# JunkyByte/deepcharuco

Hardware: AMD Instinct MI355X
Metric: frames/sec end-to-end (detect+refine) at 320x240; corner-id match vs ref (higher is better)
Workload: dtype f32; 1 GPU; bs=32/GPU x1 GPU(s) = 32 frames of 320x240, full detect+refine pipeline (BASELINE configs[1]); preset=cfg2, batch_per_gpu=32, global_batch=32, height=240, width=320, corner_pool_per_gpu=2048, frames=board, truncated_frames=0, distinct_ids_in_batch=16, parallelism=frames sharded, 1 process/GPU x1

## Files before the change

deepcharuco_amd/_lib.py:

```python
from __future__ import annotations

import ctypes as C
import os
import subprocess
from typing import Optional

_HERE = os.path.dirname(os.path.abspath(__file__))
LIB_PATH = os.environ.get("DCX_LIB") or os.path.join(_HERE, "libdeepcharuco_amd.so")
CSRC = os.path.join(_HERE, "csrc")

_lib: Optional[C.CDLL] = None


class DcxError(RuntimeError):
    def __init__(self, code: int, where: str):
        self.code = code
        try:
            msg = lib().dcx_error_string(code).decode()
        except Exception:
            msg = "?"
        super().__init__(f"{where} failed with code {code}: {msg}")


def build(force: bool = False, verbose: bool = False) -> str:
    cmd = ["make", "-C", CSRC, "-j4"]
    if force:
        subprocess.run(["make", "-C", CSRC, "clean"], check=True, capture_output=not verbose)
    res = subprocess.run(cmd, capture_output=True, text=True)
    if res.returncode != 0:
        raise RuntimeError("building libdeepcharuco_amd.so failed:\n" + res.stdout[-4000:] + res.stderr[-8000:])
    if verbose:
        print(res.stdout)
    return LIB_PATH


_vp, _i, _l, _sz = C.c_void_p, C.c_int, C.c_long, C.c_size_t

SIGNATURES = {
    "dcx_version": (C.c_char_p, []),
    "dcx_error_string": (C.c_char_p, [_i]),
    "dcx_detector_create": (_i, [C.POINTER(_vp), C.POINTER(_vp), _i, _i]),
    "dcx_detector_destroy": (_i, [_vp]),
    "dcx_refiner_create": (_i, [C.POINTER(_vp), C.POINTER(_vp), _i]),
    "dcx_refiner_destroy": (_i, [_vp]),
    "dcx_detector_workspace_bytes": (_sz, [_vp, _i, _i, _i]),
    "dcx_refiner_workspace_bytes": (_sz, [_vp, _i]),
    "dcx_bgr2gray": (_i, [_vp, _l, _i, _i, _i, _i, _vp, _vp]),
    "dcx_bgr2gray_legacy14": (_i, [_vp, _l, _i, _i, _i, _i, _vp, _vp]),
    "dcx_pre_image": (_i, [_vp, _vp, _sz, _vp]),
    "dcx_detector_forward": (_i, [_vp, _vp, _l, _i, _vp, _i, _i, _i, _vp, _sz, _vp, _vp, _vp]),
    "dcx_detector_decode": (_i, [_vp, _i, _i, _i, _vp, _i, _i, _vp, _vp, _vp, _vp, _vp]),
    "dcx_pred_to_keypoints": (_i, [_vp, _vp, _i, _i, _i, _i, _i, _i, _i, _vp, _vp, _vp, _vp, _vp]),
    "dcx_label_to_keypoints": (_i, [_vp, _vp, _i, _i, _i, _i, _i, _vp, _vp, _vp, _vp, _vp]),
    "dcx_build_patch_table": (_i, [_vp, _vp, _i, _i, _vp, _vp, _vp]),
    "dcx_extract_patches_u8": (_i, [_vp, _l, _i, _i, _i, _vp, _vp, _i, _vp, _vp]),
    "dcx_extract_patches_f32": (_i, [_vp, _i, _i, _vp, _vp, _i, _vp, _vp]),
    "dcx_refiner_forward": (_i, [_vp, _vp, _i, _vp, _vp, _vp, _sz, _vp, _vp, _vp, _vp]),
    "dcx_argmax2d": (_i, [_vp, _i, _i, _i, _vp, _vp]),
    "dcx_pipeline_workspace_bytes": (_sz, [_vp, _vp, _i, _i, _i, _i]),
    "dcx_infer_batch": (_i, [_vp, _vp, _vp, _l, _i, _i, _i, _i, _i, _i, _i, _vp, _sz, _vp, _vp, _vp, _vp, _vp, _vp]),
    "dcx_stream_synchronize": (_i, [_vp]),
    "dcx_solve_pnp_pool": (_i, [_vp, _vp, _vp, _vp, _i, _i, _i, _i, C.c_double, C.POINTER(C.c_double), C.POINTER(C.c_double), _i,
                               _vp, _vp, _vp]),
    "dcx_solve_pnp_ransac_workspace_bytes": (_sz, [_i, _i, _i]),
    "dcx_solve_pnp_ransac_pool": (_i, [_vp, _vp, _vp, _vp, _i, _i, _i, _i, C.c_double, C.POINTER(C.c_double), C.POINTER(C.c_double), _i,
                                      _i, C.c_double, _i, C.c_uint, _vp, _sz, _vp, _vp, _vp, _vp, _vp]),
    "dcx_calibrate_workspace_bytes": (_sz, [_i]),
    "dcx_calibrate_pool": (_i, [_vp, _vp, _vp, _vp, _i, _i, _i, _i, C.c_double, _i, _i, _vp, _sz, _vp, _vp,
                               C.POINTER(C.c_double), _vp]),
    "dcx_conv_layer": (_i, [_vp, _i, _i, _i, _i, _vp, _vp, _vp, _vp, _vp, _vp, _i, _i, _i, _i, _i, _i, _vp, _vp]),
    "dcx_nchw_to_c4": (_i, [_vp, _i, _i, _i, _i, _vp, _vp]),
    "dcx_c4_to_nchw": (_i, [_vp, _i, _i, _i, _i, _vp, _vp]),
    "dcx_set_timing": (_i, [_i]),
    "dcx_get_timing": (_i, []),
    "dcx_profile_enabled": (_i, []),
    "dcx_last_timings": (_i, [C.POINTER(C.c_float)]),
    "dcx_conv_pick_name": (C.c_char_p, [_i] * 8),
    "dcx_conv_pick_name_ups": (C.c_char_p, [_i] * 9),
    "dcx_set_deterministic": (_i, [_i]),
    "dcx_get_deterministic": (_i, []),
    "dcx_calibrate_xcd": (_i, [_i, C.POINTER(C.c_float), _vp]),
    "dcx_set_xcd_weights": (_i, [C.POINTER(C.c_float)]),
    "dcx_get_xcd_weights": (_i, [C.POINTER(C.c_float)]),
    "dcx_set_tail_fence": (_i, [_i]),
    "dcx_get_tail_fence": (_i, []),
    "dcx_profile_enable": (_i, [_i]),
    "dcx_profile_count": (_i, []),
    "dcx_profile_filter": (_i, [_i]),
    "dcx_profile_sample": (_i, [_i]),
    "dcx_profile_fetch": (_i, [C.POINTER(_i), C.POINTER(_i), C.POINTER(_i), C.POINTER(C.c_double), C.POINTER(C.c_float), _i]),
    "dcx_profile_kernel_name": (C.c_char_p, [_i]),
    "dcx_profile_clocks": (_i, [C.POINTER(C.c_float), _i]),
    "dcx_profile_probe_words": (_i, [_i, C.POINTER(C.c_ulonglong)]),
}


def lib() -> C.CDLL:
    global _lib
    if _lib is None:
        if not os.path.exists(LIB_PATH):
            raise RuntimeError(
                f"{LIB_PATH} not found: build it with `python -c 'import __graft_entry__ as g; g.build()'` "
                f"or `make -C {CSRC}`. deepcharuco_amd has no CPU / stock-PyTorch fallback.")
        handle = C.CDLL(LIB_PATH)
        for name, (res, args) in SIGNATURES.items():
            fn = getattr(handle, name)
            fn.restype = res
            fn.argtypes = args
        _lib = handle
    return _lib


def csrc_sha256() -> str:
    import hashlib
    h = hashlib.sha256()
    for name in sorted(os.listdir(CSRC)):
        if name.endswith((".hip", ".h")):
            with open(os.path.join(CSRC, name), "rb") as f:
                h.update(name.encode())
                h.update(f.read())
    return h.hexdigest()


def check(rc: int, where: str) -> None:
    if rc != 0:
        raise DcxError(rc, where)


def ptr(t) -> Optional[int]:
    if t is None:
        return None
    return t.data_ptr()


def current_stream() -> int:
    import torch
    return torch.cuda.current_stream().cuda_stream
```

deepcharuco_amd/csrc/dcx_api.hip:

```cpp
#include "dcx_common.h"

#include <math.h>
#include <stdlib.h>
#include <string.h>
#include <new>
#include <vector>

namespace {

constexpr float kBnEps = 1e-5f;

inline size_t align_up(size_t v, size_t a) { return (v + a - 1) / a * a; }


std::vector<float> pack_conv(const float* w, int cout, int cin, int ks, int cout_pad) {
    const int taps = ks * ks, cq = cin / 4;
    std::vector<float> out((size_t)taps * cq * cout_pad * 4, 0.0f);
    for (int o = 0; o < cout; ++o)
        for (int i = 0; i < cin; ++i)
            for (int t = 0; t < taps; ++t)
                out[(((size_t)t * cq + (i >> 2)) * cout_pad + o) * 4 + (i & 3)] = w[((size_t)o * cin + i) * taps + t];
    return out;
}

std::vector<float> pack_conv_wino2(const float* w, int cout, int cin, int cout_pad) {
    const int cq = cin / 4;
    std::vector<float> out((size_t)16 * cq * cout_pad * 4, 0.0f);
    for (int o = 0; o < cout; ++o)
        for (int i = 0; i < cin; ++i) {
            const float* g = w + ((size_t)o * cin + i) * 9;
            float h[4][3], u[4][4];
            for (int kx = 0; kx < 3; ++kx) {
                const float g0 = g[kx], g1 = g[3 + kx], g2 = g[6 + kx];
                h[0][kx] = g0; h[1][kx] = ((g0 + g1) + g2) * 0.5f; h[2][kx] = ((g0 - g1) + g2) * 0.5f; h[3][kx] = g2;
            }
            for (int xi = 0; xi < 4; ++xi) {
                u[xi][0] = h[xi][0]; u[xi][1] = ((h[xi][0] + h[xi][1]) + h[xi][2]) * 0.5f;
                u[xi][2] = ((h[xi][0] - h[xi][1]) + h[xi][2]) * 0.5f; u[xi][3] = h[xi][2];
            }
            for (int pos = 0; pos < 16; ++pos)
                out[(((size_t)pos * cq + (i >> 2)) * cout_pad + o) * 4 + (i & 3)] = u[pos >> 2][pos & 3];
        }
    return out;
}

std::vector<float> pack_conv_ups2(const float* w, int cout, int cin, int cout_pad) {
    const int cq = cin / 4;
    std::vector<float> out((size_t)16 * cq * cout_pad * 4, 0.0f);
    static const int lo[2][2] = {{0, 1}, {0, 2}}, hi[2][2] = {{0, 2}, {1, 2}};
    for (int o = 0; o < cout; ++o)
        for (int i = 0; i < cin; ++i) {
            const float* g = w + ((size_t)o * cin + i) * 9;
            for (int ph = 0; ph < 4; ++ph)
                for (int tap = 0; tap < 4; ++tap) {
                    const int a = ph >> 1, b = ph & 1, dy = tap >> 1, dx = tap & 1;
                    float r[3];
                    for (int kx = 0; kx < 3; ++kx) {
                        r[kx] = g[lo[a][dy] * 3 + kx];
                        for (int ky = lo[a][dy] + 1; ky <= hi[a][dy]; ++ky) r[kx] = r[kx] + g[ky * 3 + kx];
                    }
                    float v = r[lo[b][dx]];
                    for (int kx = lo[b][dx] + 1; kx <= hi[b][dx]; ++kx) v = v + r[kx];
                    out[(((size_t)(ph * 4 + tap) * cq + (i >> 2)) * cout_pad + o) * 4 + (i & 3)] = v;
                }
        }
    return out;
}

std::vector<float> pack_conv_ups2w(const float* w, int cout, int cin, int cout_pad) {
    const int cq = cin / 4;
    const std::vector<float> ph = pack_conv_ups2(w, cout, cin, cout_pad);
    std::vector<float> out((size_t)36 * cq * cout_pad * 4, 0.0f);
    const size_t plane = (size_t)cq * cout_pad * 4;
    for (int p = 0; p < 4; ++p)
        for (size_t e = 0; e < plane; ++e) {
            float wc[2][3];
            for (int dy = 0; dy < 2; ++dy) {
                const float g0 = ph[(size_t)(p * 4 + dy * 2 + 0) * plane + e], g1 = ph[(size_t)(p * 4 + dy * 2 + 1) * plane + e];
                wc[dy][0] = g0; wc[dy][1] = g0 + g1; wc[dy][2] = g1;
            }
            for (int nu = 0; nu < 3; ++nu) {
                out[(size_t)(p * 9 + 0 * 3 + nu) * plane + e] = wc[0][nu];
                out[(size_t)(p * 9 + 1 * 3 + nu) * plane + e] = wc[0][nu] + wc[1][nu];
                out[(size_t)(p * 9 + 2 * 3 + nu) * plane + e] = wc[1][nu];
            }
        }
    return out;
}

void fold_bn(const float* gamma, const float* bbeta, const float* mean, const float* var, int c, int c_pad,
             std::vector<float>& alpha, std::vector<float>& beta) {
    alpha.assign(c_pad, 0.0f);
    beta.assign(c_pad, 0.0f);
    for (int i = 0; i < c; ++i) {
        const float inv = 1.0f / sqrtf(var[i] + kBnEps);
        const float a = gamma[i] * inv;
        alpha[i] = a;
        beta[i] = bbeta[i] - mean[i] * a;
    }
}

std::vector<float> pad_vec(const float* v, int c, int c_pad) {
    std::vector<float> out(c_pad, 0.0f);
    memcpy(out.data(), v, sizeof(float) * c);
    return out;
}

struct DevLayer {
    float* w = nullptr;
    float* w_wino2 = nullptr;
    float* w_ups2w = nullptr;
    float* bias = nullptr;
    float* alpha = nullptr;
    float* beta = nullptr;
    int cin = 0, cout = 0, cout_pad = 0, ks = 3;
};

int upload(const std::vector<float>& h, float** d) {
    DCX_CHECK_HIP(hipMalloc((void**)d, h.size() * sizeof(float)));
    DCX_CHECK_HIP(hipMemcpy(*d, h.data(), h.size() * sizeof(float), hipMemcpyHostToDevice));
    return 0;
}

void free_layer(DevLayer& l) {
    if (l.w) (void)hipFree(l.w);
    if (l.w_wino2) (void)hipFree(l.w_wino2);
    if (l.w_ups2w) (void)hipFree(l.w_ups2w);
    if (l.bias) (void)hipFree(l.bias);
    if (l.alpha) (void)hipFree(l.alpha);
    if (l.beta) (void)hipFree(l.beta);
    l = DevLayer();
}

struct HostConv {
    const float* w; const float* b;
    const float* g; const float* be; const float* mu; const float* var;
};

int make_layer(const HostConv& h, int cin, int cout, int ks, DevLayer* out, bool ups_input = false) {
    DevLayer l;
    l.cin = cin; l.cout = cout; l.ks = ks;
    l.cout_pad = dcx_conv_cout_pad(cout);
    int rc = upload(pack_conv(h.w, cout, cin, ks, l.cout_pad), &l.w);
    if (rc == 0) rc = upload(pad_vec(h.b, cout, l.cout_pad), &l.bias);
    if (rc == 0 && h.g != nullptr) {
        std::vector<float> al, be;
        fold_bn(h.g, h.be, h.mu, h.var, cout, l.cout_pad, al, be);
        for (int i = 0; i < cout; ++i) be[i] = fmaf(h.b[i], al[i], be[i]);
        rc = upload(al, &l.alpha);
        if (rc == 0) rc = upload(be, &l.beta);
        if (rc == 0 && ks == 3) rc = upload(pack_conv_wino2(h.w, cout, cin, l.cout_pad), &l.w_wino2);
        if (rc == 0 && ks == 3 && ups_input) rc = upload(pack_conv_ups2w(h.w, cout, cin, l.cout_pad), &l.w_ups2w);
    }
    if (rc != 0) { free_layer(l); return rc; }
    *out = l;
    return 0;
}

int make_first_layer(const HostConv& h, DevLayer* out) {
    DevLayer l;
    l.cin = 1; l.cout = 64; l.cout_pad = 64; l.ks = 3;
    std::vector<float> w(9 * 64);
    for (int o = 0; o < 64; ++o)
        for (int t = 0; t < 9; ++t) w[t * 64 + o] = h.w[o * 9 + t];
    std::vector<float> al, be;
    fold_bn(h.g, h.be, h.mu, h.var, 64, 64, al, be);
    int rc = upload(w, &l.w);
    if (rc == 0) rc = upload(pad_vec(h.b, 64, 64), &l.bias);
    if (rc == 0) rc = upload(al, &l.alpha);
    if (rc == 0) rc = upload(be, &l.beta);
    if (rc != 0) { free_layer(l); return rc; }
    *out = l;
    return 0;
}

bool g_timing = false;
hipEvent_t g_ev[5];
bool g_ev_ok = false;
int timing_mark(int i, hipStream_t s) {
    if (!g_timing) return 0;
    if (!g_ev_ok) {
        for (auto& e : g_ev) DCX_CHECK_HIP(hipEventCreate(&e));
        g_ev_ok = true;
    }
    DCX_CHECK_HIP(hipEventRecord(g_ev[i], s));
    return 0;
}

}

struct dcx_detector {
    int n_ids = 16;
    DevLayer first;
    DevLayer enc[7];
    DevLayer heads_a;
    DevLayer head_loc, head_ids;
};

struct dcx_refiner {
    DevLayer first;
    DevLayer mid[9];
    DevLayer head_a;
    float* head_w = nullptr;
    float head_b = 0.f;
};

namespace {

struct DetWs {
    size_t buf0, buf1, loc, ids, codes, conf, total;
    int ids_quads;
};
DetWs det_layout(int n_ids, int b, int h, int w) {
    DetWs L;
    const size_t hw = (size_t)h * w, cells = (size_t)(h / 8) * (w / 8);
    L.ids_quads = (n_ids + 1 + 3) / 4;
    size_t off = 0;
    L.buf0 = off; off = align_up(off + (size_t)b * 64 * hw * 4, 256);
    L.buf1 = off; off = align_up(off + (size_t)b * 16 * hw * 4, 256);
    L.loc = off;  off = align_up(off + (size_t)b * 68 * cells * 4, 256);
    L.ids = off;  off = align_up(off + (size_t)b * L.ids_quads * 4 * cells * 4, 256);
    L.codes = off; off = align_up(off + (size_t)b * cells * 4, 256);
    L.conf = off; off = align_up(off + (size_t)b * cells * 8, 256);
    L.total = off;
    return L;
}

struct RefWs {
    size_t buf0, buf1, pval, pidx, total;
};
constexpr int kRefTiles = 32;
RefWs ref_layout(int p) {
    RefWs L;
    size_t off = 0;
    L.buf0 = off; off = align_up(off + (size_t)p * 65536 * 4, 256);
    L.buf1 = off; off = align_up(off + (size_t)p * 65536 * 4, 256);
    L.pval = off; off = align_up(off + (size_t)p * kRefTiles * 4, 256);
    L.pidx = off; off = align_up(off + (size_t)p * kRefTiles * 4, 256);
    L.total = off;
    return L;
}

DcxConvArgs conv_args(const DevLayer& l, const float* in, int n, int in_cq_total, int in_cq_off, int hin, int win,
                      int ups, int pad, float* out, int out_cq_total, const int* n_limit) {
    DcxConvArgs a;
    memset(&a, 0, sizeof(a));
    a.in = in; a.w = l.w; a.w_wino2 = l.w_wino2; a.w_ups2w = l.w_ups2w; a.bias = l.bias; a.alpha = l.alpha; a.beta = l.beta; a.out = out;
    a.n_limit = n_limit;
    a.n = n; a.in_cq_total = in_cq_total; a.in_cq_off = in_cq_off; a.cin = l.cin;
    a.hin = hin; a.win = win; a.ups = ups; a.pad = pad;
    a.ho = (hin << ups) + 2 * pad - (l.ks - 1);
    a.wo = (win << ups) + 2 * pad - (l.ks - 1);
    a.out_cq_total = out_cq_total; a.out_cq_off = 0;
    a.cout_pad = l.cout_pad; a.cout_quads = (l.cout + 3) / 4; a.cout_real = l.cout;
    return a;
}

}

extern "C" const char* dcx_version(void) { return "deepcharuco_amd 0.1 (gfx950, fp32 MFMA)"; }

extern "C" const char* dcx_error_string(int code) {
    switch (code) {
        case 0: return "ok";
        case DCX_E_ARG: return "DCX_E_ARG: null pointer or bad scalar argument";
        case DCX_E_SHAPE: return "DCX_E_SHAPE: unsupported shape (H/W below 8, patches not 24x24, batch x kmax too large, ...)";
        case DCX_E_WS: return "DCX_E_WS: workspace too small";
        case DCX_E_NIDS: return "DCX_E_NIDS: n_ids outside [1, 62] or dust_bin outside [0, 255]";
        default: return code > 0 ? hipGetErrorString((hipError_t)code) : "unknown dcx error";
    }
}

extern "C" int dcx_detector_create(dcx_detector** out, const float* const* t, int n_tensors, int n_ids) {
    if (!out || !t) return DCX_E_ARG;
    if (n_ids < 1 || n_ids > 62) return DCX_E_NIDS;
    if (n_tensors != 64) return DCX_E_ARG;
    for (int i = 0; i < n_tensors; ++i)
        if (!t[i]) return DCX_E_ARG;
    if (const int rc = dcx_xcd_init()) return rc;
    dcx_detector* d = new (std::nothrow) dcx_detector();
    if (!d) return (int)hipErrorOutOfMemory;
    d->n_ids = n_ids;
    auto hc = [&](int base, bool bn) {
        return HostConv{t[base], t[base + 1], bn ? t[base + 2] : nullptr, bn ? t[base + 3] : nullptr,
                        bn ? t[base + 4] : nullptr, bn ? t[base + 5] : nullptr};
    };
    static const int enc_cin[7] = {64, 64, 64, 64, 128, 128, 128};
    static const int enc_cout[7] = {64, 64, 64, 128, 128, 128, 128};
    int rc = make_first_layer(hc(0, true), &d->first);
    for (int i = 0; rc == 0 && i < 7; ++i) rc = make_layer(hc(6 + 6 * i, true), enc_cin[i], enc_cout[i], 3, &d->enc[i]);
    if (rc == 0) {
        const HostConv pa = hc(48, true), da = hc(56, true);
        const size_t wsz = (size_t)256 * 128 * 9;
        std::vector<float> w(2 * wsz), b(512), g(512), be(512), mu(512), var(512);
        memcpy(w.data(), pa.w, wsz * 4); memcpy(w.data() + wsz, da.w, wsz * 4);
        auto cat = [](std::vector<float>& dst, const float* x, const float* y) {
            memcpy(dst.data(), x, 256 * 4); memcpy(dst.data() + 256, y, 256 * 4);
        };
        cat(b, pa.b, da.b); cat(g, pa.g, da.g); cat(be, pa.be, da.be); cat(mu, pa.mu, da.mu); cat(var, pa.var, da.var);
        rc = make_layer(HostConv{w.data(), b.data(), g.data(), be.data(), mu.data(), var.data()}, 128, 512, 3,
                        &d->heads_a);
    }
    if (rc == 0) rc = make_layer(hc(54, false), 256, 65, 1, &d->head_loc);
    if (rc == 0) rc = make_layer(hc(62, false), 256, n_ids + 1, 1, &d->head_ids);
    if (rc != 0) { dcx_detector_destroy(d); return rc; }
    *out = d;
    return 0;
}

extern "C" int dcx_detector_destroy(dcx_detector* d) {
    if (!d) return 0;
    free_layer(d->first);
    for (auto& l : d->enc) free_layer(l);
    free_layer(d->heads_a); free_layer(d->head_loc); free_layer(d->head_ids);
    delete d;
    return 0;
}

extern "C" size_t dcx_detector_workspace_bytes(const dcx_detector* det, int batch, int height, int width) {
    if (!det || batch <= 0 || height <= 0 || width <= 0) return 0;
    return det_layout(det->n_ids, batch, height, width).total;
}

namespace {
int detector_run(const dcx_detector* det, const uint8_t* d_frames_u8, long frame_stride, int pitch, int pix,
                 const float* d_images_f32, int batch, int height, int width, void* d_ws, size_t ws_bytes,
                 bool with_heads, float* d_loc_nchw, float* d_ids_nchw, int32_t* zero_words, int n_zero, void* stream);
}

extern "C" int dcx_detector_forward(const dcx_detector* det, const uint8_t* d_frames_u8, long frame_stride, int pitch,
                                    const float* d_images_f32, int batch, int height, int width, void* d_ws,
                                    size_t ws_bytes, float* d_loc_nchw, float* d_ids_nchw, void* stream) {
    return detector_run(det, d_frames_u8, frame_stride, pitch, DCX_PIX_GRAY8, d_images_f32, batch, height, width, d_ws, ws_bytes, true,
                        d_loc_nchw, d_ids_nchw, nullptr, 0, stream);
}

namespace {
int detector_run(const dcx_detector* det, const uint8_t* d_frames_u8, long frame_stride, int pitch, int pix,
                 const float* d_images_f32, int batch, int height, int width, void* d_ws, size_t ws_bytes,
                 bool with_heads, float* d_loc_nchw, float* d_ids_nchw, int32_t* zero_words, int n_zero, void* stream) {
    if (!det || !d_ws) return DCX_E_ARG;
    if ((d_frames_u8 == nullptr) == (d_images_f32 == nullptr)) return DCX_E_ARG;
    if (batch <= 0 || height < 8 || width < 8) return DCX_E_SHAPE;
    const DetWs L = det_layout(det->n_ids, batch, height, width);
    if (ws_bytes < L.total) return DCX_E_WS;
    hipStream_t s = (hipStream_t)stream;
    char* ws = (char*)d_ws;
    float* buf0 = (float*)(ws + L.buf0);
    float* buf1 = (float*)(ws + L.buf1);
    float* loc = (float*)(ws + L.loc);
    float* ids = (float*)(ws + L.ids);
    const int h = height, w = width;
    int rc;
    const int pt0 = dcx_prof_begin(DCX_PROF_CONV1A, batch, s);
    if (d_frames_u8)
        rc = dcx_launch_conv1_u8(d_frames_u8, frame_stride, pitch, pix, batch, h, w, 1, det->first.w, det->first.bias,
                                 det->first.alpha, det->first.beta, buf0, nullptr, zero_words, n_zero, s);
    else
        rc = dcx_launch_conv1_f32(d_images_f32, (long)h * w, w, batch, h, w, 1, det->first.w, det->first.bias,
                                  det->first.alpha, det->first.beta, buf0, nullptr, s);
    if (rc) return rc;
    if ((rc = dcx_prof_end(pt0, s))) return rc;
    struct Step { int layer, div, pool; };
    static const Step steps[7] = {{0, 1, 1}, {1, 2, 0}, {2, 2, 1}, {3, 4, 0}, {4, 4, 1}, {5, 8, 0}, {6, 8, 0}};
    float* src = buf0;
    float* dst = buf1;
    for (const Step& st : steps) {
        const DevLayer& l = det->enc[st.layer];
        DcxConvArgs a = conv_args(l, src, batch, l.cin / 4, 0, h / st.div, w / st.div, 0, 1, dst, l.cout / 4, nullptr);
        rc = dcx_launch_conv_mfma(a, 3, st.pool, DCX_EPI_BNRELU, s);
        if (rc) return rc;
        float* t = src; src = dst; dst = t;
    }
    const int hc = h / 8, wc = w / 8;
    {
        DcxConvArgs a = conv_args(det->heads_a, src, batch, 32, 0, hc, wc, 0, 1, dst, 128, nullptr);
        rc = dcx_launch_conv_mfma(a, 3, 0, DCX_EPI_BNRELU, s);
        if (rc) return rc;
    }
    if (!with_heads) return 0;
    {
        DcxConvArgs a = conv_args(det->head_loc, dst, batch, 128, 0, 1, hc * wc, 0, 0, loc, 17, nullptr);
        rc = dcx_launch_conv_mfma(a, 1, 0, DCX_EPI_RAW, s);
        if (rc) return rc;
    }
    {
        DcxConvArgs a = conv_args(det->head_ids, dst, batch, 128, 64, 1, hc * wc, 0, 0, ids, L.ids_quads, nullptr);
        rc = dcx_launch_conv_mfma(a, 1, 0, DCX_EPI_RAW, s);
        if (rc) return rc;
    }
    if (d_loc_nchw) { rc = dcx_c4_to_nchw(loc, batch, 65, hc, wc, d_loc_nchw, stream); if (rc) return rc; }
    if (d_ids_nchw) { rc = dcx_c4_to_nchw(ids, batch, det->n_ids + 1, hc, wc, d_ids_nchw, stream); if (rc) return rc; }
    return 0;
}
}

extern "C" int dcx_detector_decode(const dcx_detector* det, int batch, int height, int width, void* d_ws,
                                   int dust_bin, int kmax, int32_t* d_counts, int32_t* d_rows, int32_t* d_loc_argmax,
                                   int32_t* d_ids_argmax, void* stream) {
    if (!det || !d_ws) return DCX_E_ARG;
    if (batch <= 0 || height < 8 || width < 8) return DCX_E_SHAPE;
    const DetWs L = det_layout(det->n_ids, batch, height, width);
    const int hc = height / 8, wc = width / 8;
    const long cells = (long)hc * wc;
    char* ws = (char*)d_ws;
    DcxLogitView lv{(const float*)(ws + L.loc), 17 * 4 * cells, 4 * cells, 4, 1};
    DcxLogitView iv{(const float*)(ws + L.ids), (long)L.ids_quads * 4 * cells, 4 * cells, 4, 1};
    return dcx_launch_decode(lv, iv, batch, 65, det->n_ids + 1, hc, wc, dust_bin, kmax, d_counts, d_rows,
                             d_loc_argmax, d_ids_argmax, (int32_t*)(ws + L.codes), (hipStream_t)stream);
}

extern "C" int dcx_refiner_create(dcx_refiner** out, const float* const* t, int n_tensors) {
    if (!out || !t) return DCX_E_ARG;
    if (n_tensors != 68) return DCX_E_ARG;
    for (int i = 0; i < n_tensors; ++i)
        if (!t[i]) return DCX_E_ARG;
    if (const int rc = dcx_xcd_init()) return rc;
    dcx_refiner* r = new (std::nothrow) dcx_refiner();
    if (!r) return (int)hipErrorOutOfMemory;
    auto hc = [&](int base) { return HostConv{t[base], t[base + 1], t[base + 2], t[base + 3], t[base + 4], t[base + 5]}; };
    static const int cin[9] = {64, 64, 128, 128, 128, 128, 128, 128, 64};
    static const int cout[9] = {64, 128, 128, 128, 128, 128, 128, 64, 64};
    int rc = make_first_layer(hc(0), &r->first);
    for (int i = 0; rc == 0 && i < 9; ++i) rc = make_layer(hc(6 + 6 * i), cin[i], cout[i], 3, &r->mid[i], i == 5 || i == 7);
    if (rc == 0) rc = make_layer(hc(60), 64, 64, 3, &r->head_a, true);
    if (rc == 0) {
        std::vector<float> hw(t[66], t[66] + 64);
        rc = upload(hw, &r->head_w);
        r->head_b = t[67][0];
    }
    if (rc != 0) { dcx_refiner_destroy(r); return rc; }
    *out = r;
    return 0;
}

extern "C" int dcx_refiner_destroy(dcx_refiner* r) {
    if (!r) return 0;
    free_layer(r->first);
    for (auto& l : r->mid) free_layer(l);
    free_layer(r->head_a);
    if (r->head_w) (void)hipFree(r->head_w);
    delete r;
    return 0;
}

extern "C" size_t dcx_refiner_workspace_bytes(const dcx_refiner* rf, int max_patches) {
    if (!rf || max_patches <= 0) return 0;
    return ref_layout(max_patches).total;
}

namespace {
struct FrameSrc { const uint8_t* frames; long frame_stride; int pitch, pix, height, width; };
int refiner_run(const dcx_refiner* rf, const float* d_patches, const FrameSrc* fsrc, int max_patches, int n_hint,
                const int32_t* d_total, const int32_t* d_table, void* d_ws, size_t ws_bytes, int32_t* d_corners, float* d_xy,
                float* d_heat, void* stream);
}

extern "C" int dcx_refiner_forward(const dcx_refiner* rf, const float* d_patches, int max_patches,
                                   const int32_t* d_total, const int32_t* d_table, void* d_ws, size_t ws_bytes,
                                   int32_t* d_corners, float* d_xy, float* d_heat, void* stream) {
    return refiner_run(rf, d_patches, nullptr, max_patches, 0, d_total, d_table, d_ws, ws_bytes, d_corners, d_xy, d_heat, stream);
}

namespace {
int refiner_run(const dcx_refiner* rf, const float* d_patches, const FrameSrc* fsrc, int max_patches, int n_hint,
                const int32_t* d_total, const int32_t* d_table, void* d_ws, size_t ws_bytes, int32_t* d_corners, float* d_xy,
                float* d_heat, void* stream) {
    if (!rf || !d_ws || ((d_patches == nullptr) == (fsrc == nullptr))) return DCX_E_ARG;
    if (fsrc != nullptr && (d_total == nullptr || d_table == nullptr)) return DCX_E_ARG;
    if (d_xy != nullptr && d_table == nullptr) return DCX_E_ARG;
    if (max_patches <= 0 || max_patches > (1 << 22)) return DCX_E_SHAPE;
    const RefWs L = ref_layout(max_patches);
    if (ws_bytes < L.total) return DCX_E_WS;
    hipStream_t s = (hipStream_t)stream;
    char* ws = (char*)d_ws;
    float* buf0 = (float*)(ws + L.buf0);
    float* buf1 = (float*)(ws + L.buf1);
    const int p = max_patches;
    const int* lim = d_total;
    const int pt0 = dcx_prof_begin(DCX_PROF_PATCHES, p, s);
    int rc = fsrc != nullptr
        ? dcx_launch_conv1_patches_u8(fsrc->frames, fsrc->frame_stride, fsrc->pitch, fsrc->pix, fsrc->height, fsrc->width, d_table, d_total, p, n_hint,
                                      rf->first.w, rf->first.bias, rf->first.alpha, rf->first.beta, buf0, s)
        : dcx_launch_conv1_f32(d_patches, 576, 24, p, 24, 24, 0, rf->first.w, rf->first.bias, rf->first.alpha,
                               rf->first.beta, buf0, lim, s);
    if (rc) return rc;
    if ((rc = dcx_prof_end(pt0, s))) return rc;
    struct Step { int layer, hin, ups, pad, pool; };
    static const Step steps[9] = {
        {0, 22, 0, 0, 0},
        {1, 20, 0, 0, 0},
        {2, 18, 0, 0, 1},
        {3, 8, 0, 1, 0},
        {4, 8, 0, 1, 0},
        {5, 8, 1, 1, 0},
        {6, 16, 0, 1, 0},
        {7, 16, 1, 1, 0},
        {8, 32, 0, 1, 0},
    };
    float* src = buf0;
    float* dst = buf1;
    for (const Step& st : steps) {
        const DevLayer& l = rf->mid[st.layer];
        DcxConvArgs a = conv_args(l, src, p, l.cin / 4, 0, st.hin, st.hin, st.ups, st.pad, dst, l.cout / 4, lim);
        a.n_hint = lim != nullptr ? n_hint : 0;
        rc = dcx_launch_conv_mfma(a, 3, st.pool, DCX_EPI_BNRELU, s);
        if (rc) return rc;
        float* t = src; src = dst; dst = t;
    }
    int heat_tiles = 0;
    {
        DcxConvArgs a = conv_args(rf->head_a, src, p, 16, 0, 32, 32, 1, 1, nullptr, 16, lim);
        a.head_w = rf->head_w; a.head_b = rf->head_b; a.heat = d_heat;
        a.part_val = (float*)(ws + L.pval); a.part_idx = (int*)(ws + L.pidx);
        heat_tiles = dcx_conv_heat_tiles(a.ho, a.wo, a.w_ups2w != nullptr ? 1 : 0);
        if (heat_tiles <= 0 || heat_tiles > kRefTiles) return DCX_E_SHAPE;
        rc = dcx_launch_conv_mfma(a, 3, 0, DCX_EPI_HEAT, s);
        if (rc) return rc;
    }
    const int pt1 = dcx_prof_begin(DCX_PROF_FINALIZE, p, s);
    rc = dcx_launch_refine_finalize((const float*)(ws + L.pval), (const int*)(ws + L.pidx), heat_tiles, 64, p, lim,
                                    d_table, d_corners, d_xy, s);
    if (rc) return rc;
    return dcx_prof_end(pt1, s);
}
}

namespace {
struct PipeWs { size_t det, table, ctrl, ref, total; int ctrl_words; };
PipeWs pipe_layout(const dcx_detector* det, const dcx_refiner* rf, int b, int h, int w, int pool) {
    PipeWs L;
    size_t off = 0;
    L.det = off; off = align_up(off + det_layout(det->n_ids, b, h, w).total, 256);
    L.table = off; off = align_up(off + (size_t)pool * 16, 256);
    L.ctrl_words = 64 + b;
    L.ctrl = off; off = align_up(off + (size_t)L.ctrl_words * 4, 256);
    L.ref = off; off = align_up(off + (rf ? ref_layout(pool).total : 0), 256);
    L.total = off;
    return L;
}
}

extern "C" size_t dcx_pipeline_workspace_bytes(const dcx_detector* det, const dcx_refiner* rf, int batch, int height,
                                               int width, int pool) {
    if (!det || batch <= 0 || height <= 0 || width <= 0 || pool <= 0) return 0;
    return pipe_layout(det, rf, batch, height, width, pool).total;
}

namespace {
int infer_range(const dcx_detector* det, const dcx_refiner* rf, const uint8_t* d_frames_u8, long frame_stride, int pitch, int pix,
                int batch, int height, int width, int dust_bin, int pool, char* ws, size_t ws_bytes, int32_t* d_counts,
                int32_t* d_starts, int32_t* d_rows, float* d_xy, float* d_conf, hipStream_t s, bool timing) {
    void* stream = (void*)s;
    const PipeWs L = pipe_layout(det, rf, batch, height, width, pool);
    if (ws_bytes < L.total) return DCX_E_WS;
    int rc = timing ? timing_mark(0, s) : 0;
    if (rc) return rc;
    int32_t* ctrl = (int32_t*)(ws + L.ctrl);
    rc = detector_run(det, d_frames_u8, frame_stride, pitch, pix, nullptr, batch, height, width, ws + L.det, L.table - L.det,
                      false, nullptr, nullptr, ctrl, L.ctrl_words, stream);
    if (rc) return rc;
    if (timing && (rc = timing_mark(1, s))) return rc;
    int32_t* table = (int32_t*)(ws + L.table);
    {
        const DetWs D = det_layout(det->n_ids, batch, height, width);
        const int hc = height / 8, wc = width / 8;
        const float* act = (const float*)(ws + L.det + D.buf0);
        int32_t* codes = (int32_t*)(ws + L.det + D.codes);
        DcxPoolOut po;
        po.tickets = ctrl + 64; po.cursor = ctrl; po.counts = d_counts; po.starts = d_starts; po.rows = d_rows;
        po.table = rf ? table : nullptr; po.conf = d_conf; po.conf_cells = (float*)(ws + L.det + D.conf);
        po.wc = wc; po.pool = pool;
        const int pt = dcx_prof_begin(DCX_PROF_TAIL, batch, s);
        rc = dcx_launch_tail(act, batch, hc * wc, det->head_loc.w, det->head_loc.bias, det->head_ids.w, det->head_ids.bias,
                             det->head_ids.cout_pad, det->n_ids + 1, dust_bin, codes, nullptr, nullptr, &po, s);
        if (rc) return rc;
        if ((rc = dcx_prof_end(pt, s))) return rc;
    }
    if (timing && (rc = timing_mark(2, s))) return rc;
    if (rf == nullptr) return timing ? timing_mark(3, s) : 0;
    const long expect = (long)batch * det->n_ids;
    const FrameSrc src{d_frames_u8, frame_stride, pitch, pix, height, width};
    rc = refiner_run(rf, nullptr, &src, pool, (int)(expect < pool ? expect : pool), ctrl, table,
                     ws + L.ref, L.total - L.ref, nullptr, d_xy, nullptr, stream);
    if (rc) return rc;
    return timing ? timing_mark(3, s) : 0;
}
}

extern "C" int dcx_infer_batch(const dcx_detector* det, const dcx_refiner* rf, const uint8_t* d_frames_u8,
                               long frame_stride, int pitch, int pixel_format, int batch, int height, int width, int dust_bin,
                               int pool, void* d_ws, size_t ws_bytes, int32_t* d_counts, int32_t* d_starts, int32_t* d_rows,
                               float* d_xy, float* d_conf, void* stream) {
    if (!det || !d_frames_u8 || !d_ws || !d_counts || !d_starts || !d_rows) return DCX_E_ARG;
    if (rf != nullptr && d_xy == nullptr) return DCX_E_ARG;
    if (pixel_format != DCX_PIX_GRAY8 && pixel_format != DCX_PIX_BGR8 && pixel_format != DCX_PIX_BGR8_LEGACY14) return DCX_E_ARG;
    if (pool <= 0 || pool > (1 << 22)) return DCX_E_SHAPE;
    if (batch <= 0 || batch > (1 << 20) || height < 8 || width < 8) return DCX_E_SHAPE;
    if (pitch < width * (pixel_format == DCX_PIX_GRAY8 ? 1 : 3)) return DCX_E_SHAPE;
    if (dust_bin < 0 || dust_bin > 255) return DCX_E_NIDS;
    hipStream_t s = (hipStream_t)stream;
    char* ws = (char*)d_ws;
    return infer_range(det, rf, d_frames_u8, frame_stride, pitch, pixel_format, batch, height, width, dust_bin, pool, ws, ws_bytes,
                       d_counts, d_starts, d_rows, d_xy, d_conf, s, true);
}

extern "C" int dcx_stream_synchronize(void* stream) { return (int)hipStreamSynchronize((hipStream_t)stream); }

extern "C" int dcx_set_timing(int enabled) { g_timing = enabled != 0; return 0; }
extern "C" int dcx_get_timing(void) { return g_timing ? 1 : 0; }

extern "C" int dcx_last_timings(float* h_ms4) {
    if (!h_ms4) return DCX_E_ARG;
    if (!g_ev_ok) return DCX_E_ARG;
    DCX_CHECK_HIP(hipEventElapsedTime(&h_ms4[0], g_ev[0], g_ev[1]));
    DCX_CHECK_HIP(hipEventElapsedTime(&h_ms4[1], g_ev[1], g_ev[2]));
    DCX_CHECK_HIP(hipEventElapsedTime(&h_ms4[2], g_ev[2], g_ev[3]));
    DCX_CHECK_HIP(hipEventElapsedTime(&h_ms4[3], g_ev[0], g_ev[3]));
    return 0;
}

extern "C" int dcx_conv_layer(const float* d_in, int n, int cin, int hin, int win, const float* h_w, const float* h_b,
                              const float* h_g, const float* h_be, const float* h_mu, const float* h_var, int cout,
                              int ksize, int pad, int ups, int pool, int relu, float* d_out, void* stream) {
    if (!d_in || !h_w || !h_b || !d_out) return DCX_E_ARG;
    if (cin % 32 != 0 || (ksize != 3 && ksize != 1) || n <= 0) return DCX_E_SHAPE;
    const bool bn = h_g != nullptr;
    if (bn != (relu != 0)) return DCX_E_ARG;
    if (bn && (!h_be || !h_mu || !h_var)) return DCX_E_ARG;
    if (const int rc = dcx_xcd_init()) return rc;
    DevLayer l;
    int rc = make_layer(HostConv{h_w, h_b, h_g, h_be, h_mu, h_var}, cin, cout, ksize, &l, ups != 0);
    if (rc) return rc;
    DcxConvArgs a;
    if (ksize == 1) {
        if (pad != 0 || ups != 0 || pool != 0) { free_layer(l); return DCX_E_SHAPE; }
        a = conv_args(l, d_in, n, cin / 4, 0, 1, hin * win, 0, 0, d_out, (cout + 3) / 4, nullptr);
    } else {
        a = conv_args(l, d_in, n, cin / 4, 0, hin, win, ups, pad, d_out, (cout + 3) / 4, nullptr);
    }
    rc = dcx_launch_conv_mfma(a, ksize, pool, bn ? DCX_EPI_BNRELU : DCX_EPI_RAW, (hipStream_t)stream);
    hipError_t e = hipStreamSynchronize((hipStream_t)stream);
    free_layer(l);
    if (rc) return rc;
    return (int)e;
}
```

deepcharuco_amd/csrc/dcx_common.h:

```cpp
#pragma once
#include <hip/hip_runtime.h>
#include <stdint.h>
#include <stddef.h>

#include "../../include/deepcharuco_amd.h"

#define DCX_CHECK_HIP(expr)                              \
    do {                                                 \
        hipError_t _e = (expr);                          \
        if (_e != hipSuccess) return (int)_e;            \
    } while (0)


enum DcxEpilogue {
    DCX_EPI_BNRELU = 0,
    DCX_EPI_RAW = 1,
    DCX_EPI_HEAT = 2,
};

struct DcxConvArgs {
    const float* in;
    const float* w;
    const float* w_wino2;
    const float* w_ups2w;
    const float* bias;
    const float* alpha;
    const float* beta;
    float* out;
    const int* n_limit;
    unsigned long long* clk_probe;
    int probe_u0;
    const float* head_w;
    float head_b;
    float* heat;
    float* part_val;
    int* part_idx;
    int n;
    int n_hint;
    int in_cq_total, in_cq_off;
    int cin;
    int hin, win;
    int ups;
    int pad;
    int ho, wo;
    int out_cq_total, out_cq_off;
    int cout_pad;
    int cout_quads;
    int cout_real;
    int tiles_x, tiles_y;
    int xcd_walk;
    const int* xcd_cum;
    unsigned long long* xcd_stat;
    int ct_outer;
};

int dcx_launch_conv_mfma(DcxConvArgs a, int ks, int pool, int epi, hipStream_t stream);
int dcx_xcd_init();
int dcx_conv_cout_pad(int cout);
int dcx_conv_heat_tiles(int ho, int wo, int ups);

enum { DCX_PROF_CONV1A = 100, DCX_PROF_PATCHES = 101, DCX_PROF_TAIL = 102, DCX_PROF_FINALIZE = 103 };
int dcx_prof_begin(int kernel_id, int n, hipStream_t s);
int dcx_prof_end(int token, hipStream_t s);


int dcx_launch_conv1_u8(const uint8_t* frames, long frame_stride, int pitch, int pix, int n, int h, int w, int pad,
                        const float* w9x64, const float* bias, const float* alpha, const float* beta,
                        float* out_c4, const int* n_limit, int32_t* zero_words, int n_zero, hipStream_t s);
int dcx_launch_conv1_f32(const float* images, long image_stride, int pitch, int n, int h, int w, int pad,
                         const float* w9x64, const float* bias, const float* alpha, const float* beta,
                         float* out_c4, const int* n_limit, hipStream_t s);

struct DcxLogitView {
    const float* p;
    long sb, sq, sp, sc;
};
int dcx_launch_decode(DcxLogitView loc, DcxLogitView ids, int batch, int n_loc, int n_ids1, int hc, int wc,
                      int dust_bin, int kmax, int32_t* counts, int32_t* rows,
                      int32_t* loc_argmax, int32_t* ids_argmax, int32_t* codes_scratch, hipStream_t s);
struct DcxPoolOut {
    int32_t* tickets;
    int32_t* cursor;
    int32_t* counts;
    int32_t* starts;
    int32_t* rows;
    int32_t* table;
    float* conf;
    float* conf_cells;
    int wc, pool;
};
int dcx_launch_tail(const float* act_c4_512, int batch, int cells, const float* w_loc, const float* b_loc,
                    const float* w_ids, const float* b_ids, int ids_cout_pad, int n_ids1, int dust_bin,
                    int32_t* codes, int32_t* loc_argmax, int32_t* ids_argmax, const DcxPoolOut* po, hipStream_t s);
int dcx_launch_compact(const int32_t* codes, int batch, int hc, int wc, int dust_bin, int kmax, int32_t* counts,
                       int32_t* rows, hipStream_t s);
int dcx_launch_conv1_patches_u8(const uint8_t* frames, long frame_stride, int pitch, int pix, int h, int w, const int32_t* table,
                                const int* total, int max_patches, int n_hint, const float* w9x64, const float* bias,
                                const float* alpha, const float* beta, float* out_c4, hipStream_t s);
int dcx_launch_refine_finalize(const float* part_val, const int* part_idx, int tiles, int wo,
                               int max_patches, const int* total, const int32_t* table,
                               int32_t* corners, float* xy, hipStream_t s);
```

deepcharuco_amd/csrc/dcx_conv_mfma.hip:

```cpp
#include "dcx_conv_mfma.h"
#include "dcx_conv_wino2h.h"
#include "dcx_conv_wino2hs.h"
#include "dcx_conv_wino2p.h"
#include "dcx_conv_wino2ps.h"

#include <stdlib.h>
#include <string.h>
#include <atomic>
#include <mutex>
#include <vector>

namespace {

enum { FAM_DIRECT = 0,
       FAM_W2H = 3,
       FAM_W2P = 4 };

struct CfgEntry {
    int cout_tile, cap, th, tw, ks, pool, epi, acc_tiles;
    int inlane;
    int group;
    int fam;
    int (*launch)(DcxConvArgs, hipStream_t);
    const char* name;
};

#define DCX_CFG(WM, WN, MT, NT, TH, TW, KS, POOL, EPI)                                              \
    { WM * MT * 32, WN * NT * 32, TH, TW, KS, POOL, EPI, MT * NT, ((POOL) != 0 && MT == 1 && NT == 4) ? 1 : 0, 1, FAM_DIRECT, \
      &dcx_conv_launch_cfg<DcxConvCfg<WM, WN, MT, NT, TH, TW, KS, (POOL) != 0, EPI>>,                 \
      "dcx_conv_mfma_kernel<DcxConvCfg<" #WM "," #WN "," #MT "," #NT "," #TH "," #TW "," #KS "," #POOL "," #EPI ">>" }

#define DCX_W2HCFG(TH, TW, POOL, G)                                                                   \
    { 64, 128, TH, TW, 3, POOL, DCX_EPI_BNRELU, 8, 0, G, FAM_W2H,                                            \
      &dcx_conv_wino2h_launch_cfg<DcxWino2hCfg<TH, TW, (POOL) != 0, G>>,                                   \
      "dcx_conv_wino2h_kernel<DcxWino2hCfg<" #TH "," #TW "," #POOL "," #G ">>" }
#define DCX_W2HCFG_S(TH, TW, POOL)                                                                    \
    { 64, 64, TH, TW, 3, POOL, DCX_EPI_BNRELU, 4, 0, 1, FAM_W2H,                                             \
      &dcx_conv_wino2h_launch_cfg<DcxWino2hCfg<TH, TW, (POOL) != 0, 1, 1>>,                                \
      "dcx_conv_wino2h_kernel<DcxWino2hCfg<" #TH "," #TW "," #POOL ",1,1>>" }

#define DCX_W2HSCFG(POOL, CG)                                                                         \
    { 16 * CG, 64, 8, 8, 3, POOL, DCX_EPI_BNRELU, 1, 0, 1, FAM_W2H,                                          \
      &dcx_conv_wino2hs_launch_cfg<DcxWino2hsCfg<(POOL) != 0, CG>>,                                        \
      "dcx_conv_wino2hs_kernel<DcxWino2hsCfg<" #POOL "," #CG ">>" }

#define DCX_W2PCFG(TH, TW, EPI, G)                                                                    \
    { 64, 128, TH, TW, 3, 0, EPI, 5, 0, G, FAM_W2P,                                                          \
      &dcx_conv_wino2p_launch_cfg<DcxWino2pCfg<TH, TW, EPI, G>>,                                           \
      "dcx_conv_wino2p_kernel<DcxWino2pCfg<" #TH "," #TW "," #EPI "," #G ">>" }

#define DCX_W2PSCFG(CG)                                                                               \
    { 16 * CG, 64, 8, 8, 3, 0, DCX_EPI_BNRELU, 1, 0, 1, FAM_W2P,                                             \
      &dcx_conv_wino2ps_launch_cfg<DcxWino2psCfg<CG>>,                                                     \
      "dcx_conv_wino2ps_kernel<DcxWino2psCfg<" #CG ">>" }

const CfgEntry kCfgs[] = {
    DCX_CFG(1, 4, 2, 2, 8, 32, 3, 0, DCX_EPI_BNRELU),
    DCX_CFG(2, 2, 1, 1, 8, 8, 3, 0, DCX_EPI_BNRELU),
    DCX_CFG(2, 2, 1, 1, 8, 8, 3, 1, DCX_EPI_BNRELU),
    DCX_CFG(2, 2, 1, 4, 8, 32, 3, 1, DCX_EPI_BNRELU),
    DCX_CFG(1, 4, 2, 2, 1, 256, 1, 0, DCX_EPI_RAW),
    DCX_CFG(1, 4, 2, 2, 8, 32, 3, 0, DCX_EPI_HEAT),
    DCX_W2HCFG(8, 16, 0, 1),
    DCX_W2HCFG(8, 16, 1, 1),
    DCX_W2HCFG(6, 20, 0, 1),
    DCX_W2HCFG(6, 20, 1, 1),
    DCX_W2HCFG(8, 8, 0, 2),
    DCX_W2HCFG_S(8, 8, 0),
    DCX_W2HCFG_S(8, 8, 1),
    DCX_W2HSCFG(0, 4), DCX_W2HSCFG(0, 2), DCX_W2HSCFG(0, 1),
    DCX_W2HSCFG(1, 4), DCX_W2HSCFG(1, 2), DCX_W2HSCFG(1, 1),
    DCX_W2PCFG(8, 16, DCX_EPI_BNRELU, 1),
    DCX_W2PCFG(8, 16, DCX_EPI_HEAT, 1),
    DCX_W2PCFG(8, 8, DCX_EPI_BNRELU, 2),
    DCX_W2PSCFG(4), DCX_W2PSCFG(2), DCX_W2PSCFG(1),
};

int g_deterministic = -1;
int dcx_deterministic_enabled() {
    if (g_deterministic < 0) g_deterministic = dcx_env_knob(DCX_KNOB_DETERMINISTIC) ? 1 : 0;
    return g_deterministic;
}

int family_of(int cin, int cout_pad, int ks, int pool, int epi, int ups_phase) {
    if (dcx_deterministic_enabled() || ks != 3 || epi == DCX_EPI_RAW || cin < 2 * DCX_CCH) return FAM_DIRECT;
    if (ups_phase && !pool && (epi == DCX_EPI_BNRELU || (epi == DCX_EPI_HEAT && cout_pad == 64))) return FAM_W2P;
    if (epi == DCX_EPI_BNRELU) return FAM_W2H;
    return FAM_DIRECT;
}

const CfgEntry* pick(int n, int cin, int ho, int wo, int cout_pad, int ks, int pool, int epi, int allow_group = 1, int ups = 0) {
    const CfgEntry* best = nullptr;
    double best_cost = 0.0;
    const int n_cu = dcx_device_cu_count();
    auto can_run = [&](const CfgEntry& c) {
        if (c.ks != ks || c.pool != pool || c.epi != epi || cout_pad % c.cout_tile != 0) return false;
        if (c.fam == FAM_W2P) return ups == 1 && cin >= 2 * DCX_CCH && (epi != DCX_EPI_HEAT || cout_pad == 64) &&
                                     (c.group == 1 || (ho <= 2 * c.th && wo <= 2 * c.tw));
        if (c.fam == FAM_W2H) return cin >= 2 * DCX_CCH && (c.group == 1 || (allow_group && ups == 0 && ho <= c.th && wo <= c.tw));
        return true;
    };
    const char* force = getenv("DCX_FORCE_CFG");
    if (force != nullptr && force[0] != 0) {
        for (const CfgEntry& c : kCfgs)
            if (strcmp(c.name, force) == 0 && can_run(c)) return &c;
    }
    const int fam = family_of(cin, cout_pad, ks, pool, epi, ups);
    const int units = cin / DCX_CCH;
    for (const CfgEntry& c : kCfgs) {
        if (c.fam != fam || !can_run(c)) continue;
        const int ph = c.fam == FAM_W2P ? 2 : 1;
        const long tiles = (long)((ho / ph + c.th - 1) / c.th) * ((wo / ph + c.tw - 1) / c.tw);
        const long items = (long)((n + c.group - 1) / c.group) * (cout_pad / c.cout_tile) * tiles * (ph * ph);
        const double rounds = (double)((items + n_cu - 1) / n_cu);
        double cost;
        if (c.fam == FAM_W2H) {
            double item_cost = (double)units * (64 * 64.0 + (c.tw == 20 ? 700.0 : 560.0)) + 2600.0;
            if (c.acc_tiles == 4)
                item_cost = (double)units * (32 * 64.0 + 600.0) + 2000.0;
            if (c.acc_tiles == 1) {
                const int w2hs = dcx_env_knob(DCX_KNOB_W2HS);
                const int w2hs_rounds = dcx_env_knob(DCX_KNOB_W2HS_ROUNDS);
                if (!(w2hs & (c.cout_tile / 16)) || items > (long)w2hs_rounds * n_cu) continue;
                item_cost = (double)units * (8 * 64.0 * (c.cout_tile / 16) + 400.0) + 1200.0;
                if (w2hs_rounds > 1 && items > n_cu) item_cost *= 0.8;
            }
            cost = rounds * item_cost * (1.0 + 1e-6 * (double)items);
        } else if (c.fam == FAM_W2P) {
            double item_cost = (double)units * (72 * 32.0 + 500.0) + 2400.0;
            if (c.acc_tiles == 1) {
                const int w2ps = dcx_env_knob(DCX_KNOB_W2PS);
                if (!(w2ps & (c.cout_tile / 16)) || items > n_cu) continue;
                item_cost = (double)units * (12 * 32.0 * ((3 * (c.cout_tile / 16) + 3) / 4) + 400.0) + 1200.0;
            }
            cost = rounds * item_cost * (1.0 + 1e-6 * (double)items);
        } else {
            const int steps = ks * ks * (DCX_CCH / 8);
            const double item_cost = (double)units * steps * (4 * c.acc_tiles) * 64.0 + units * 520.0
                                   + c.acc_tiles * 16 * (c.inlane ? 35.0 : (pool ? 60.0 : 40.0));
            cost = rounds * item_cost;
            if (c.cout_tile == 64 && c.cap == 256) cost *= 0.999;
        }
        if (best == nullptr || cost < best_cost) { best_cost = cost; best = &c; }
    }
    return best;
}

struct ProfRec { int kernel_id, n, limited; double flops_per_image; hipEvent_t e0, e1; int slot; };
unsigned long long* g_clk_dev = nullptr;
constexpr int kClkSlots = 1024;
constexpr int kClkWords = 64;
bool g_prof = false;
int g_prof_filter = -1;
int g_prof_every = 1;
long g_prof_seen = 0;
std::vector<ProfRec> g_recs;
std::vector<hipEvent_t> g_pool;
size_t g_pool_used = 0;

hipEvent_t prof_event() {
    if (g_pool_used == g_pool.size()) {
        hipEvent_t e;
        if (hipEventCreate(&e) != hipSuccess) return nullptr;
        g_pool.push_back(e);
    }
    return g_pool[g_pool_used++];
}

}

extern "C" const char* dcx_conv_pick_name(int n, int cin, int ho, int wo, int cout, int ks, int pool, int epi) {
    const CfgEntry* c = pick(n, cin, ho, wo, dcx_conv_cout_pad(cout), ks, pool, epi);
    return c ? c->name : "";
}
extern "C" const char* dcx_conv_pick_name_ups(int n, int cin, int ho, int wo, int cout, int ks, int pool, int epi, int ups) {
    const CfgEntry* c = pick(n, cin, ho, wo, dcx_conv_cout_pad(cout), ks, pool, epi, ups == 0, ups);
    return c ? c->name : "";
}

extern "C" int dcx_set_deterministic(int enabled) { g_deterministic = enabled ? 1 : 0; return 0; }
extern "C" int dcx_get_deterministic(void) { return dcx_deterministic_enabled(); }

extern "C" int dcx_profile_enable(int enabled) {
    g_prof = enabled != 0;
    if (g_prof) { g_recs.clear(); g_pool_used = 0; }
    return 0;
}
extern "C" int dcx_profile_enabled(void) { return g_prof ? 1 : 0; }
extern "C" int dcx_profile_filter(int kernel_id) { g_prof_filter = kernel_id; return 0; }
extern "C" int dcx_profile_sample(int every) { g_prof_every = every > 1 ? every : 1; g_prof_seen = 0; return 0; }
extern "C" int dcx_profile_count(void) { return (int)g_recs.size(); }
extern "C" const char* dcx_profile_kernel_name(int id) {
    const int n = (int)(sizeof(kCfgs) / sizeof(kCfgs[0]));
    switch (id) {
        case DCX_PROF_CONV1A: return "dcx_conv1_kernel (detector conv1a)";
        case DCX_PROF_PATCHES: return "dcx_conv1_patches_kernel (RefineNet conv1a + patch gather)";
        case DCX_PROF_TAIL: return "dcx_tail_kernel (1x1 heads + arg-max + compaction)";
        case DCX_PROF_FINALIZE: return "dcx_refine_finalize_kernel";
        default: break;
    }
    return id >= 0 && id < n ? kCfgs[id].name : "?";
}

int dcx_prof_begin(int kernel_id, int n, hipStream_t stream) {
    if (!g_prof || g_prof_filter >= 0) return -1;
    ProfRec r;
    r.kernel_id = kernel_id; r.n = n; r.limited = 0; r.flops_per_image = 0.0;
    r.e0 = prof_event();
    r.e1 = prof_event();
    r.slot = (int)g_recs.size();
    if (!r.e0 || !r.e1 || hipEventRecord(r.e0, stream) != hipSuccess) return -1;
    g_recs.push_back(r);
    return r.slot;
}
int dcx_prof_end(int token, hipStream_t stream) {
    if (token < 0 || token >= (int)g_recs.size()) return 0;
    DCX_CHECK_HIP(hipEventRecord(g_recs[token].e1, stream));
    return 0;
}
extern "C" int dcx_profile_probe_words(int record, unsigned long long* out64) {
    if (!out64 || record < 0 || record >= kClkSlots || g_clk_dev == nullptr) return DCX_E_ARG;
    DCX_CHECK_HIP(hipMemcpy(out64, g_clk_dev + (size_t)kClkWords * record, kClkWords * 8, hipMemcpyDeviceToHost));
    return 0;
}

extern "C" int dcx_profile_clocks(float* ghz, int max_records) {
    if (!ghz) return DCX_E_ARG;
    const int n = (int)g_recs.size() < max_records ? (int)g_recs.size() : max_records;
    std::vector<unsigned long long> h((size_t)kClkWords * kClkSlots, 0ull);
    if (g_clk_dev != nullptr) DCX_CHECK_HIP(hipMemcpy(h.data(), g_clk_dev, h.size() * 8, hipMemcpyDeviceToHost));
    for (int i = 0; i < n; ++i) {
        ghz[i] = 0.f;
        if (i < kClkSlots) {
            const unsigned long long* p = &h[(size_t)kClkWords * i];
            if (p[3] > p[1]) ghz[i] = (float)((double)(p[2] - p[0]) / (double)(p[3] - p[1]) * 0.1);
        }
    }
    return n;
}

extern "C" int dcx_profile_fetch(int* kernel_ids, int* n_images, int* limited, double* flops_per_image, float* ms,
                                 int max_records) {
    if (!kernel_ids || !n_images || !limited || !flops_per_image || !ms) return DCX_E_ARG;
    int k = 0;
    for (const ProfRec& r : g_recs) {
        if (k >= max_records) break;
        float t = 0.f;
        if (hipEventElapsedTime(&t, r.e0, r.e1) != hipSuccess) t = -1.f;
        kernel_ids[k] = r.kernel_id; n_images[k] = r.n; limited[k] = r.limited;
        flops_per_image[k] = r.flops_per_image; ms[k] = t;
        ++k;
    }
    return k;
}

int dcx_conv_cout_pad(int cout) { return cout <= 64 ? 64 : (cout + 127) / 128 * 128; }

int dcx_current_device() {
    int dev = 0;
    if (hipGetDevice(&dev) != hipSuccess || dev < 0) dev = 0;
    return dev < DCX_MAX_DEVICES ? dev : DCX_MAX_DEVICES - 1;
}

int dcx_device_cu_count() {
    static int cus[DCX_MAX_DEVICES] = {};
    const int dev = dcx_current_device();
    if (cus[dev] == 0) {
        int v = 0;
        if (hipDeviceGetAttribute(&v, hipDeviceAttributeMultiprocessorCount, dev) == hipSuccess && v > 0)
            cus[dev] = v;
        else
            cus[dev] = 256;
    }
    return cus[dev];
}

int dcx_env_knob(DcxKnob k) {
    static struct { const char* name; int unset; bool read; int value; } knobs[DCX_KNOB_COUNT] = {
        {"DCX_DETERMINISTIC", 0},
        {"DCX_XCD_WALK", 1},
        {"DCX_OCC", 0},
        {"DCX_CT_OUTER", -1},
        {"DCX_W2HS", 7},
        {"DCX_W2HS_ROUNDS", 1},
        {"DCX_W2PS", 7},
        {"DCX_PROBE_U0", 0},
    };
    if (!knobs[k].read) { const char* e = getenv(knobs[k].name); knobs[k].value = e ? atoi(e) : knobs[k].unset; knobs[k].read = true; }
    return knobs[k].value;
}

namespace {
constexpr int kXcdTables = 256;
std::mutex g_xcd_mutex;
int* g_xcd_tab[DCX_MAX_DEVICES] = {};
int g_xcd_next[DCX_MAX_DEVICES] = {};
std::atomic<const int*> g_xcd_cur[DCX_MAX_DEVICES] = {};
float g_xcd_w[DCX_MAX_DEVICES][8];
int xcd_set_locked(int dev, const float* w8) {
    if (g_xcd_tab[dev] == nullptr)
        DCX_CHECK_HIP(hipMalloc((void**)&g_xcd_tab[dev], sizeof(int) * 16 * kXcdTables));
    double sum = 0.0;
    for (int x = 0; x < 8; ++x) { g_xcd_w[dev][x] = w8 ? w8[x] : 1.0f; sum += g_xcd_w[dev][x]; }
    double acc = 0.0;
    int cum[16] = {};
    for (int x = 0; x < 8; ++x) {
        g_xcd_w[dev][x] = (float)(g_xcd_w[dev][x] / sum);
        acc += g_xcd_w[dev][x];
        cum[x + 1] = x == 7 ? 65536 : (int)(acc * 65536.0 + 0.5);
    }
    int* slot = g_xcd_tab[dev] + 16 * (g_xcd_next[dev]++ % kXcdTables);
    DCX_CHECK_HIP(hipMemcpy(slot, cum, sizeof(cum), hipMemcpyHostToDevice));
    g_xcd_cur[dev].store(slot, std::memory_order_release);
    return 0;
}
int xcd_set(int dev, const float* w8) {
    std::lock_guard<std::mutex> lk(g_xcd_mutex);
    return xcd_set_locked(dev, w8);
}
}

int dcx_xcd_init() {
    const int dev = dcx_current_device();
    std::lock_guard<std::mutex> lk(g_xcd_mutex);
    return g_xcd_cur[dev].load(std::memory_order_relaxed) != nullptr ? 0 : xcd_set_locked(dev, nullptr);
}

int dcx_fill_xcd_cum(DcxConvArgs& a) {
    a.xcd_cum = g_xcd_cur[dcx_current_device()].load(std::memory_order_acquire);
    return a.xcd_cum != nullptr ? 0 : (int)hipErrorNotInitialized;
}

extern "C" int dcx_set_xcd_weights(const float* w8) {
    if (w8 != nullptr) {
        double sum = 0.0;
        for (int x = 0; x < 8; ++x) { if (!(w8[x] > 0.f)) return DCX_E_ARG; sum += w8[x]; }
        for (int x = 0; x < 8; ++x) { const double r = 8.0 * w8[x] / sum; if (r < 0.75 || r > 1.25) return DCX_E_ARG; }
    }
    return xcd_set(dcx_current_device(), w8);
}
extern "C" int dcx_get_xcd_weights(float* w8) {
    if (!w8) return DCX_E_ARG;
    const int rc = dcx_xcd_init();
    if (rc) return rc;
    const int dev = dcx_current_device();
    std::lock_guard<std::mutex> lk(g_xcd_mutex);
    for (int x = 0; x < 8; ++x) w8[x] = 8.0f * g_xcd_w[dev][x];
    return 0;
}

namespace {
__global__ void dcx_fill_hash_kernel(float* __restrict__ p, size_t n, float lo, float scale) {
    for (size_t i = (size_t)blockIdx.x * blockDim.x + threadIdx.x; i < n; i += (size_t)gridDim.x * blockDim.x) {
        unsigned h = (unsigned)i * 2654435761u;
        h ^= h >> 15; h *= 2246822519u; h ^= h >> 13;
        p[i] = lo + scale * (float)(h >> 8) * (1.0f / 16777216.0f);
    }
}
}

extern "C" int dcx_calibrate_xcd(int rounds, float* w8_out, void* stream) {
    if (rounds < 1 || rounds > 64) return DCX_E_ARG;
    hipStream_t s = (hipStream_t)stream;
    const int n = 32, c = 64, h = 240, w = 320;
    const size_t in_elems = (size_t)n * c * h * w, out_elems = in_elems / 4, w_elems = (size_t)16 * c * c;
    float *d_in = nullptr, *d_out = nullptr, *d_w = nullptr, *d_ab = nullptr;
    unsigned long long* d_stat = nullptr;
    auto cleanup = [&]() { (void)hipFree(d_in); (void)hipFree(d_out); (void)hipFree(d_w); (void)hipFree(d_ab); (void)hipFree(d_stat); };
    hipError_t e = hipMalloc((void**)&d_in, in_elems * 4);
    if (e == hipSuccess) e = hipMalloc((void**)&d_out, out_elems * 4);
    if (e == hipSuccess) e = hipMalloc((void**)&d_w, w_elems * 4);
    if (e == hipSuccess) e = hipMalloc((void**)&d_ab, 3 * c * 4);
    if (e == hipSuccess) e = hipMalloc((void**)&d_stat, 17 * 8);
    if (e == hipSuccess) e = hipMemsetD32Async((hipDeviceptr_t)d_ab, 0x3f800000, 3 * c, s);
    if (e != hipSuccess) { cleanup(); return (int)e; }
    hipLaunchKernelGGL(dcx_fill_hash_kernel, dim3(4096), dim3(256), 0, s, d_in, in_elems, -1.0f, 2.0f);
    hipLaunchKernelGGL(dcx_fill_hash_kernel, dim3(64), dim3(256), 0, s, d_w, w_elems, -0.05f, 0.1f);
    if ((e = hipGetLastError()) != hipSuccess) { cleanup(); return (int)e; }
    DcxConvArgs a;
    memset(&a, 0, sizeof(a));
    a.in = d_in; a.w = d_w; a.w_wino2 = d_w; a.bias = d_ab; a.alpha = d_ab + c; a.beta = d_ab + 2 * c; a.out = d_out;
    a.n = n; a.in_cq_total = c / 4; a.cin = c; a.hin = h; a.win = w; a.pad = 1; a.ho = h; a.wo = w;
    a.out_cq_total = c / 4; a.cout_pad = c; a.cout_quads = c / 4; a.cout_real = c;
    const int dev = dcx_current_device();
    float keep[8];
    {
        std::lock_guard<std::mutex> lk(g_xcd_mutex);
        for (int x = 0; x < 8; ++x) keep[x] = g_xcd_cur[dev].load(std::memory_order_relaxed) != nullptr ? g_xcd_w[dev][x] : 0.125f;
        const int rc = xcd_set_locked(dev, nullptr);
        if (rc) { cleanup(); return rc; }
    }
    double speed[8] = {};
    int rc = 0, used = 0;
    for (int r = 0; r < rounds + 2 && rc == 0; ++r) {
        if ((e = hipMemsetAsync(d_stat, 0, 17 * 8, s)) != hipSuccess) { rc = (int)e; break; }
        a.xcd_stat = r >= 2 ? d_stat : nullptr;
        rc = dcx_launch_conv_mfma(a, 3, 1, DCX_EPI_BNRELU, s);
        if (rc != 0 || r < 2) continue;
        unsigned long long hst[17];
        if ((e = hipMemcpyAsync(hst, d_stat, sizeof(hst), hipMemcpyDeviceToHost, s)) != hipSuccess || (e = hipStreamSynchronize(s)) != hipSuccess) { rc = (int)e; break; }
        bool ok = hst[8] != 0;
        double dur[8];
        for (int x = 0; x < 8 && ok; ++x) {
            ok = hst[9 + x] > 0;
            if (ok) { dur[x] = (double)hst[x] / (double)hst[9 + x] - (double)hst[8]; ok = dur[x] > 0.0; }
        }
        if (!ok) continue;
        for (int x = 0; x < 8; ++x) speed[x] += 1.0 / dur[x];
        ++used;
    }
    (void)hipStreamSynchronize(s);
    cleanup();
    if (rc == 0 && used > 0) {
        float w8[8];
        for (int x = 0; x < 8; ++x) w8[x] = (float)(speed[x] / used);
        rc = dcx_set_xcd_weights(w8);
    } else if (rc == 0) {
        rc = DCX_E_SHAPE;
    }
    if (rc != 0) (void)xcd_set(dev, keep);
    if (rc == 0 && w8_out != nullptr) (void)dcx_get_xcd_weights(w8_out);
    return rc;
}

int dcx_conv_heat_tiles(int ho, int wo, int ups) {
    const CfgEntry* c = pick(1 << 20, 64, ho, wo, 64, 3, 0, DCX_EPI_HEAT, 1, ups);
    if (c == nullptr) return 0;
    if (c->fam == FAM_W2P) return 4 * ((ho / 2 + c->th - 1) / c->th) * ((wo / 2 + c->tw - 1) / c->tw);
    return ((ho + c->th - 1) / c->th) * ((wo + c->tw - 1) / c->tw);
}

int dcx_launch_conv_mfma(DcxConvArgs a, int ks, int pool, int epi, hipStream_t stream) {
    if (a.in == nullptr || a.w == nullptr || a.bias == nullptr) return DCX_E_ARG;
    if (epi != DCX_EPI_HEAT && a.out == nullptr) return DCX_E_ARG;
    if (epi != DCX_EPI_RAW && (a.alpha == nullptr || a.beta == nullptr)) return DCX_E_ARG;
    if (pool && (a.ho < 2 || a.wo < 2)) return DCX_E_SHAPE;
    const CfgEntry* c = pick(epi == DCX_EPI_HEAT ? (1 << 20) : (a.n_hint > 0 && a.n_hint < a.n ? a.n_hint : a.n), a.cin, a.ho, a.wo, a.cout_pad, ks, pool, epi,
                             a.ups == 0 && a.pad == 1,
                             (a.ups == 1 && a.pad == 1 && ks == 3 && a.w_ups2w != nullptr) ? 1 : 0);
    if (c == nullptr) return DCX_E_SHAPE;
    if (!g_prof || (g_prof_filter >= 0 && g_prof_filter != (int)(c - kCfgs))) return c->launch(a, stream);
    if (g_prof_every > 1 && (g_prof_seen++ % g_prof_every) != 0) return c->launch(a, stream);
    ProfRec r;
    r.kernel_id = (int)(c - kCfgs);
    r.n = a.n;
    r.limited = a.n_limit != nullptr;
    r.flops_per_image = 2.0 * a.cout_real * a.cin * ks * ks
                      * (double)a.ho * a.wo;
    r.e0 = prof_event();
    r.e1 = prof_event();
    r.slot = (int)g_recs.size();
    if (g_clk_dev == nullptr) {
        if (hipMalloc((void**)&g_clk_dev, sizeof(unsigned long long) * kClkWords * kClkSlots) != hipSuccess) g_clk_dev = nullptr;
        else (void)hipMemset(g_clk_dev, 0, sizeof(unsigned long long) * kClkWords * kClkSlots);
    }
    if (g_clk_dev != nullptr && r.slot < kClkSlots) a.clk_probe = g_clk_dev + (size_t)kClkWords * r.slot;
    a.probe_u0 = dcx_env_knob(DCX_KNOB_PROBE_U0);
    if (!r.e0 || !r.e1) return (int)hipErrorOutOfMemory;
    DCX_CHECK_HIP(hipEventRecord(r.e0, stream));
    const int rc = c->launch(a, stream);
    DCX_CHECK_HIP(hipEventRecord(r.e1, stream));
    if (rc == 0) g_recs.push_back(r);
    return rc;
}
```

deepcharuco_amd/csrc/dcx_conv_shared.h:

```cpp
#pragma once
#include "dcx_common.h"

typedef float dcx_f32x16 __attribute__((ext_vector_type(16)));
typedef float dcx_f32x4 __attribute__((ext_vector_type(4)));
typedef float dcx_f32x2 __attribute__((ext_vector_type(2)));
typedef unsigned int dcx_u32x4 __attribute__((ext_vector_type(4)));

#define DCX_CCH 16

__device__ __forceinline__ float4 dcx_f4_zero() { return make_float4(0.f, 0.f, 0.f, 0.f); }

__device__ __forceinline__ float dcx_vmax(float x, float y) {
    float r;
    asm("v_max_f32 %0, %1, %2" : "=v"(r) : "v"(x), "v"(y));
    return r;
}
__device__ __forceinline__ dcx_f32x2 dcx_pk_add(dcx_f32x2 x, dcx_f32x2 y) {
    dcx_f32x2 r;
    asm("v_pk_add_f32 %0, %1, %2" : "=v"(r) : "v"(x), "v"(y));
    return r;
}
__device__ __forceinline__ dcx_f32x2 dcx_pk_sub(dcx_f32x2 x, dcx_f32x2 y) {
    dcx_f32x2 r;
    asm("v_pk_add_f32 %0, %1, %2 neg_lo:[0,1] neg_hi:[0,1]" : "=v"(r) : "v"(x), "v"(y));
    return r;
}
__device__ __forceinline__ float4 dcx_sub4(const float4& x, const float4& y) {
    const dcx_f32x2 lo = dcx_pk_sub(dcx_f32x2{x.x, x.y}, dcx_f32x2{y.x, y.y}), hi = dcx_pk_sub(dcx_f32x2{x.z, x.w}, dcx_f32x2{y.z, y.w});
    return make_float4(lo.x, lo.y, hi.x, hi.y);
}
__device__ __forceinline__ float4 dcx_add4(const float4& x, const float4& y) {
    const dcx_f32x2 lo = dcx_pk_add(dcx_f32x2{x.x, x.y}, dcx_f32x2{y.x, y.y}), hi = dcx_pk_add(dcx_f32x2{x.z, x.w}, dcx_f32x2{y.z, y.w});
    return make_float4(lo.x, lo.y, hi.x, hi.y);
}
__device__ __forceinline__ float4 dcx_fmas4(const float4& x, const dcx_f32x2 s, const float4& y) {
    const dcx_f32x2 lo = __builtin_elementwise_fma(dcx_f32x2{x.x, x.y}, s, dcx_f32x2{y.x, y.y});
    const dcx_f32x2 hi = __builtin_elementwise_fma(dcx_f32x2{x.z, x.w}, s, dcx_f32x2{y.z, y.w});
    return make_float4(lo.x, lo.y, hi.x, hi.y);
}
__device__ __forceinline__ float4 dcx_fma4(float4 x, float4 al, float4 be) {
    const dcx_f32x2 lo = __builtin_elementwise_fma(dcx_f32x2{x.x, x.y}, dcx_f32x2{al.x, al.y}, dcx_f32x2{be.x, be.y});
    const dcx_f32x2 hi = __builtin_elementwise_fma(dcx_f32x2{x.z, x.w}, dcx_f32x2{al.z, al.w}, dcx_f32x2{be.z, be.w});
    return make_float4(lo.x, lo.y, hi.x, hi.y);
}
#define DCX_VMAX0(x) asm volatile("v_max_f32 %0, 0, %0" : "+v"(x))
#define DCX_MAX_DPP(x, PERM) asm volatile("v_max_f32_dpp %0, %0, %0 quad_perm:" PERM " row_mask:0xf bank_mask:0xf" : "+v"(x))
__device__ __forceinline__ float4 dcx_relu_quad_max(float4 v) {
    DCX_VMAX0(v.x); DCX_VMAX0(v.y); DCX_VMAX0(v.z); DCX_VMAX0(v.w);
    DCX_MAX_DPP(v.x, "[1,0,3,2]"); DCX_MAX_DPP(v.y, "[1,0,3,2]"); DCX_MAX_DPP(v.z, "[1,0,3,2]"); DCX_MAX_DPP(v.w, "[1,0,3,2]");
    DCX_MAX_DPP(v.x, "[2,3,0,1]"); DCX_MAX_DPP(v.y, "[2,3,0,1]"); DCX_MAX_DPP(v.z, "[2,3,0,1]"); DCX_MAX_DPP(v.w, "[2,3,0,1]");
    return v;
}

constexpr unsigned DCX_OOB = 0x80000000u;
__device__ __forceinline__ float4 dcx_buffer_load_f4(__amdgpu_buffer_rsrc_t rsrc, unsigned voff, unsigned soff = 0) {
    const dcx_u32x4 v = __builtin_amdgcn_raw_buffer_load_b128(rsrc, voff, soff, 0);
    return make_float4(__uint_as_float(v.x), __uint_as_float(v.y), __uint_as_float(v.z), __uint_as_float(v.w));
}

struct DcxItem {
    int n, ct, ty, tx;
    int ph;
};
__device__ __forceinline__ DcxItem dcx_decode_item(int wi, int tiles_x, int tiles_y, int n_ct) {
    DcxItem it;
    it.tx = wi % tiles_x; wi /= tiles_x;
    it.ty = wi % tiles_y; wi /= tiles_y;
    it.ct = wi % n_ct;
    it.n = wi / n_ct;
    it.ph = 0;
    return it;
}
__device__ __forceinline__ DcxItem dcx_decode_item_phases(int wi, int tiles_x, int tiles_y, int n_ct) {
    DcxItem it;
    it.ph = wi & 3; wi >>= 2;
    it.tx = wi % tiles_x; wi /= tiles_x;
    it.ty = wi % tiles_y; wi /= tiles_y;
    it.ct = wi % n_ct;
    it.n = wi / n_ct;
    return it;
}

__device__ __forceinline__ int dcx_n_eff(const DcxConvArgs& a) {
    int n_eff = a.n;
    if (a.n_limit != nullptr) n_eff = min(n_eff, *a.n_limit);
    return n_eff;
}
__device__ __forceinline__ int dcx_xcd_bound(int total, int x, int cum) {
    const int eq = (int)(((long)total * x) >> 3);
    const int dev = (int)(((long)total * (cum - (x << 13))) >> 16);
    return eq + ((dev + (dev >= 0 ? 16 : -16)) / 32) * 32;
}
struct DcxWalk { int w, w_end, gstride; };
__device__ __forceinline__ DcxWalk dcx_item_walk(const DcxConvArgs& a, int total) {
    int w = blockIdx.x, w_end = total, gstride = gridDim.x;
    if (a.xcd_walk && (gridDim.x & 7) == 0) {
        const int x = blockIdx.x & 7;
        const int lo = dcx_xcd_bound(total, x, a.xcd_cum[x]);
        w_end = dcx_xcd_bound(total, x + 1, a.xcd_cum[x + 1]);
        gstride = gridDim.x >> 3;
        w = lo + (blockIdx.x >> 3);
    }
    return {w, w_end, gstride};
}

__device__ __forceinline__ void dcx_probe_ends(const DcxConvArgs& a, int tid, int word) {
    if (a.clk_probe != nullptr && blockIdx.x == 0 && tid == 0) {
        a.clk_probe[word] = __builtin_amdgcn_s_memtime();
        a.clk_probe[word + 1] = __builtin_amdgcn_s_memrealtime();
    }
}

__device__ __forceinline__ int dcx_f23_a(int xi) { return xi == 0 ? 0 : xi == 2 ? 2 : 1; }
__device__ __forceinline__ int dcx_f23_b(int xi) { return xi == 2 ? 1 : xi == 3 ? 3 : 2; }
__device__ __forceinline__ float dcx_f23_sgn(int xi) { return xi == 1 ? 1.f : -1.f; }
template <class T> __device__ __forceinline__ T dcx_at23(int i, int xi) { return i == 0 ? (xi < 3 ? T(1) : T(0)) : (xi == 0 ? T(0) : xi == 1 ? T(1) : T(-1)); }

constexpr int DCX_MAX_DEVICES = 64;
int dcx_current_device();
int dcx_device_cu_count();
int dcx_fill_xcd_cum(DcxConvArgs& a);
enum DcxKnob { DCX_KNOB_DETERMINISTIC, DCX_KNOB_XCD_WALK, DCX_KNOB_OCC, DCX_KNOB_CT_OUTER, DCX_KNOB_W2HS, DCX_KNOB_W2HS_ROUNDS,
               DCX_KNOB_W2PS, DCX_KNOB_PROBE_U0, DCX_KNOB_COUNT };
int dcx_env_knob(DcxKnob k);

template <void (*KERNEL)(const DcxConvArgs)>
static int dcx_launch_persistent(DcxConvArgs& a, long items, int threads, int occ, bool honour_dcx_occ, size_t lds_bytes, int max_dyn_lds,
                                 hipStream_t stream, void (*after_walk)(DcxConvArgs&) = nullptr) {
    if (items <= 0 || items > 0x7fffffffL) return DCX_E_SHAPE;
    if (honour_dcx_occ) {
        const int occ_env = dcx_env_knob(DCX_KNOB_OCC);
        if (occ_env > 0 && occ_env < occ) occ = occ_env;
    }
    const long resident = (long)occ * dcx_device_cu_count();
    const long blocks = items < resident ? items : resident;
    a.xcd_walk = dcx_env_knob(DCX_KNOB_XCD_WALK) && blocks == resident && (resident & 7) == 0 ? 1 : 0;
    if (const int rc = dcx_fill_xcd_cum(a)) return rc;
    if (after_walk != nullptr) after_walk(a);
    static bool attr_set[DCX_MAX_DEVICES] = {};
    const int dev_i = dcx_current_device();
    if (!attr_set[dev_i]) {
        DCX_CHECK_HIP(hipFuncSetAttribute(reinterpret_cast<const void*>(KERNEL), hipFuncAttributeMaxDynamicSharedMemorySize, max_dyn_lds));
        attr_set[dev_i] = true;
    }
    if (lds_bytes > 160 * 1024) return DCX_E_SHAPE;
    hipLaunchKernelGGL(KERNEL, dim3((unsigned)blocks), dim3(threads), lds_bytes, stream, a);
    return (int)hipGetLastError();
}
```

deepcharuco_amd/csrc/dcx_tail.hip:

```cpp
#include "dcx_common.h"

int dcx_device_cu_count();

#include <stdlib.h>
#include <string.h>

typedef float dcx_t_f32x16 __attribute__((ext_vector_type(16)));

namespace {

constexpr int kTailPF = 2;
#ifndef DCX_TAIL_PF_SMALL
#define DCX_TAIL_PF_SMALL 8
#endif
constexpr int kTailPFSmall = DCX_TAIL_PF_SMALL;

__device__ __forceinline__ int dcx_ld_agent(const int32_t* p) {
    return __hip_atomic_load(const_cast<int32_t*>(p), __ATOMIC_RELAXED, __HIP_MEMORY_SCOPE_AGENT);
}
template <bool CONF>
__device__ __forceinline__ void dcx_tail_compact_frame(const int32_t* codes, int cells, int dust_bin, int b, const DcxPoolOut& po,
                                                       int* s_cnt , int* s_bcast) {
    const int tid = threadIdx.x, lane = tid & 63, wave = tid >> 6;
    const int nsuper = (cells + 2047) / 2048;
    const int32_t* fc = codes + (size_t)b * cells;
    const int idle = dust_bin << 8;
    int total = 0;
    if (nsuper > 1) {
        int c = 0;
        for (int i = tid; i < cells; i += 256) c += ((dcx_ld_agent(fc + i) >> 8) != dust_bin) ? 1 : 0;
#pragma unroll
        for (int off = 32; off >= 1; off >>= 1) c += __shfl_xor(c, off);
        if (lane == 0) s_cnt[wave] = c;
        __syncthreads();
        total = s_cnt[0] + s_cnt[1] + s_cnt[2] + s_cnt[3];
        __syncthreads();
    }
    int run = 0, start = 0;
    for (int sc = 0; sc < nsuper; ++sc) {
        int code[8];
#pragma unroll
        for (int c = 0; c < 8; ++c) {
            const int cell = sc * 2048 + c * 256 + tid;
            code[c] = cell < cells ? dcx_ld_agent(fc + cell) : idle;
        }
        unsigned long long m[8];
#pragma unroll
        for (int c = 0; c < 8; ++c) {
            m[c] = __ballot((code[c] >> 8) != dust_bin);
            if (lane == 0) s_cnt[c * 4 + wave] = __popcll(m[c]);
        }
        __syncthreads();
        int base[8], acc = 0;
#pragma unroll
        for (int c = 0; c < 8; ++c) {
            const int w0 = s_cnt[c * 4], w1 = s_cnt[c * 4 + 1], w2 = s_cnt[c * 4 + 2], w3 = s_cnt[c * 4 + 3];
            base[c] = acc + (wave > 0 ? w0 : 0) + (wave > 1 ? w1 : 0) + (wave > 2 ? w2 : 0);
            acc += w0 + w1 + w2 + w3;
        }
        if (sc == 0) {
            if (nsuper == 1) total = acc;
            if (tid == 0) {
                const int st = atomicAdd(po.cursor, total);
                po.counts[b] = total;
                po.starts[b] = st;
                *s_bcast = st;
            }
            __syncthreads();
            start = *s_bcast;
        }
#pragma unroll
        for (int c = 0; c < 8; ++c) {
            if ((code[c] >> 8) != dust_bin) {
                const int pos = start + run + base[c] + __popcll(m[c] & ((1ull << lane) - 1ull));
                if (pos < po.pool) {
                    const int cell = sc * 2048 + c * 256 + tid;
                    const int la = code[c] & 255, ia = code[c] >> 8;
                    const int cy = cell / po.wc, cx = cell - cy * po.wc;
                    const int x = 8 * cx + (la & 7);
                    const int y = 8 * cy + (la >> 3);
                    reinterpret_cast<int4*>(po.rows)[pos] = make_int4(x, y, ia, cell);
                    if (po.table) reinterpret_cast<int4*>(po.table)[pos] = make_int4(b, x, y, pos);
                    if (CONF && po.conf) {
                        const unsigned long long cv = __hip_atomic_load(reinterpret_cast<unsigned long long*>(po.conf_cells) + (size_t)b * cells + cell,
                                                                        __ATOMIC_RELAXED, __HIP_MEMORY_SCOPE_AGENT);
                        reinterpret_cast<unsigned long long*>(po.conf)[pos] = cv;
                    }
                }
            }
        }
        run += acc;
        __syncthreads();
    }
}

template <int NT, int IDS_TILES, bool CONF, int PF = kTailPF>
__global__ __launch_bounds__(256) void dcx_tail_kernel(const float4* __restrict__ act, int act_cq_total, int cells,
                                                        const float4* __restrict__ w_loc, const float* __restrict__ b_loc,
                                                        const float4* __restrict__ w_ids, const float* __restrict__ b_ids,
                                                        int ids_cout_pad, int n_ids1, int tiles_per_frame, int dust_bin,
                                                        int32_t* codes, int32_t* __restrict__ loc_argmax,
                                                        int32_t* __restrict__ ids_argmax, DcxPoolOut po, int fence) {
#if defined(__HIP_DEVICE_COMPILE__) && !defined(__gfx950__) && !defined(__gfx942__)
#error "dcx_tail_kernel's fence-free hand-off counts on gfx942 / gfx950 behaviour (stores are tracked by vmcnt; sc1 stores / loads are write-through / L2-bypassing at agent scope): build with DCX_TAIL_FENCE semantics reviewed for any other ISA"
#endif
    constexpr int NPIX = 32 * NT;
    __shared__ float red_v[4 + 1][NPIX];
    __shared__ int red_i[4 + 1][NPIX];
    __shared__ float red_s[CONF ? 4 + 1 : 1][NPIX];
    __shared__ int s_cnt[32];
    __shared__ int s_bcast, s_last;
    const int tid = threadIdx.x, lane = tid & 63, wave = tid >> 6;
    const int half = lane >> 5, l31 = lane & 31;
    const int item = blockIdx.x;
    const int b = item / tiles_per_frame;
    const int cell0 = (item - b * tiles_per_frame) * NPIX;
    const bool is_ids = wave == 3;
    const int jobs = is_ids ? IDS_TILES : 1;
    const float4* wq = is_ids ? w_ids : w_loc;
    const int cout_pad = is_ids ? ids_cout_pad : 128;
    const int cq_base = is_ids ? 64 : 0;
    const int n_valid = is_ids ? n_ids1 : 65;
    const float* bias = is_ids ? b_ids : b_loc;

    size_t a_off[NT];
#pragma unroll
    for (int nt = 0; nt < NT; ++nt) {
        const int pix = min(cell0 + nt * 32 + l31, cells - 1);
        a_off[nt] = ((size_t)b * act_cq_total + cq_base + half) * (size_t)cells + pix;
    }
    const size_t k_stride = (size_t)2 * cells;

    for (int job = 0; job < jobs; ++job) {
        const int m0 = is_ids ? job * 32 : wave * 32;
        const size_t w_lane = (size_t)half * cout_pad + (m0 + l31);
        const size_t w_stride = (size_t)2 * cout_pad;
        dcx_t_f32x16 acc[NT];
#pragma unroll
        for (int nt = 0; nt < NT; ++nt)
#pragma unroll
            for (int r = 0; r < 16; ++r) acc[nt][r] = 0.f;
        float4 aq[32 + PF], bq[32 + PF][NT];
#pragma unroll
        for (int st = 0; st < PF; ++st) {
            aq[st] = wq[w_lane + st * w_stride];
#pragma unroll
            for (int nt = 0; nt < NT; ++nt) bq[st][nt] = act[a_off[nt] + st * k_stride];
        }
#pragma unroll
        for (int st = 0; st < 32; ++st) {
            __builtin_amdgcn_sched_barrier(0);
            if (st + PF < 32) {
                aq[st + PF] = wq[w_lane + (st + PF) * w_stride];
#pragma unroll
                for (int nt = 0; nt < NT; ++nt) bq[st + PF][nt] = act[a_off[nt] + (st + PF) * k_stride];
            }
            __builtin_amdgcn_sched_barrier(0);
            const float4 av = aq[st];
#pragma unroll
            for (int j = 0; j < 4; ++j) {
                const float a1 = j == 0 ? av.x : j == 1 ? av.y : j == 2 ? av.z : av.w;
#pragma unroll
                for (int nt = 0; nt < NT; ++nt) {
                    const float4 bv = bq[st][nt];
                    const float b1 = j == 0 ? bv.x : j == 1 ? bv.y : j == 2 ? bv.z : bv.w;
                    acc[nt] = __builtin_amdgcn_mfma_f32_32x32x2f32(a1, b1, acc[nt], 0, 0, 0);
                }
            }
        }
#pragma unroll
        for (int nt = 0; nt < NT; ++nt) {
            float best = -INFINITY;
            int besti = 0x7fffffff;
            float lv[16];
#pragma unroll
            for (int r = 0; r < 16; ++r) {
                const int co = m0 + 8 * (r >> 2) + 4 * half + (r & 3);
                lv[r] = -INFINITY;
                if (co < n_valid) {
                    const float v = acc[nt][r] + bias[co];
                    lv[r] = v;
                    if (v > best || besti == 0x7fffffff) { best = v; besti = co; }
                }
            }
            float ssum = 0.f;
            if (CONF && besti != 0x7fffffff) {
#pragma unroll
                for (int r = 0; r < 16; ++r) ssum += lv[r] == -INFINITY ? 0.f : expf(lv[r] - best);
            }
            const float ov = __shfl_xor(best, 32);
            const int oi = __shfl_xor(besti, 32);
            const float os = CONF ? __shfl_xor(ssum, 32) : 0.f;
            const float mine = best;
            if (oi != 0x7fffffff && (besti == 0x7fffffff || ov > best || (ov == best && oi < besti))) { best = ov; besti = oi; }
            if (half == 0) {
                const int slot = is_ids ? 3 + job : wave;
                red_v[slot][nt * 32 + l31] = best;
                red_i[slot][nt * 32 + l31] = besti;
                if (CONF) {
                    const float a = ssum == 0.f ? 0.f : ssum * expf(mine - best);
                    const float c = os == 0.f ? 0.f : os * expf(ov - best);
                    red_s[slot][nt * 32 + l31] = a + c;
                }
            }
        }
    }
    __syncthreads();
    if (tid < NPIX) {
        const int cell = cell0 + tid;
        if (cell < cells) {
            float lv = red_v[0][tid];
            int la = red_i[0][tid];
#pragma unroll
            for (int t = 1; t < 3; ++t) {
                const int ti = red_i[t][tid];
                if (ti != 0x7fffffff && red_v[t][tid] > lv) { lv = red_v[t][tid]; la = ti; }
            }
            float iv = red_v[3][tid];
            int ia = red_i[3][tid];
            if (IDS_TILES > 1) {
                const int ti = red_i[4][tid];
                if (ti != 0x7fffffff && red_v[4][tid] > iv) { iv = red_v[4][tid]; ia = ti; }
            }
            const size_t o = (size_t)b * cells + cell;
            if (CONF) {
                float sl = 0.f, si = 0.f;
#pragma unroll
                for (int t = 0; t < 3; ++t)
                    if (red_i[t][tid] != 0x7fffffff) sl += red_s[t][tid] * expf(red_v[t][tid] - lv);
                si = red_s[3][tid] * expf(red_v[3][tid] - iv);
                if (IDS_TILES > 1 && red_i[4][tid] != 0x7fffffff) si += red_s[4][tid] * expf(red_v[4][tid] - iv);
                const float2 cf2 = make_float2(1.0f / sl, 1.0f / si);
                __hip_atomic_store(reinterpret_cast<unsigned long long*>(po.conf_cells) + o, *reinterpret_cast<const unsigned long long*>(&cf2),
                                   __ATOMIC_RELAXED, __HIP_MEMORY_SCOPE_AGENT);
            }
            if (la == 64) ia = dust_bin;
            __hip_atomic_store(codes + o, la | (ia << 8), __ATOMIC_RELAXED, __HIP_MEMORY_SCOPE_AGENT);
            if (loc_argmax) loc_argmax[o] = la;
            if (ids_argmax) ids_argmax[o] = ia;
        }
    }
    if (po.tickets == nullptr) return;
    if (fence) __threadfence();
    else asm volatile("s_waitcnt vmcnt(0)" ::: "memory");
    __syncthreads();
    if (tid == 0) s_last = __hip_atomic_fetch_add(&po.tickets[b], 1, fence ? __ATOMIC_ACQ_REL : __ATOMIC_RELAXED, __HIP_MEMORY_SCOPE_AGENT) == tiles_per_frame - 1;
    __syncthreads();
    if (!s_last) return;
    if (fence) __threadfence();
    dcx_tail_compact_frame<CONF>(codes, cells, dust_bin, b, po, s_cnt, &s_bcast);
}

}

static int g_tail_fence = -1;
static int dcx_tail_fence_mode() {
    if (g_tail_fence < 0) { const char* e = getenv("DCX_TAIL_FENCE"); g_tail_fence = (e && atoi(e)) ? 1 : 0; }
    return g_tail_fence;
}
extern "C" int dcx_set_tail_fence(int enabled) { g_tail_fence = enabled ? 1 : 0; return 0; }
extern "C" int dcx_get_tail_fence(void) { return dcx_tail_fence_mode(); }

int dcx_launch_tail(const float* act, int batch, int cells, const float* w_loc, const float* b_loc, const float* w_ids,
                    const float* b_ids, int ids_cout_pad, int n_ids1, int dust_bin, int32_t* codes, int32_t* loc_argmax,
                    int32_t* ids_argmax, const DcxPoolOut* po_in, hipStream_t s) {
    if (!act || !w_loc || !b_loc || !w_ids || !b_ids || !codes) return DCX_E_ARG;
    if (batch <= 0 || cells <= 0 || n_ids1 < 2 || n_ids1 > 64 || ids_cout_pad < n_ids1) return DCX_E_SHAPE;
    if (dust_bin < 0 || dust_bin > 255) return DCX_E_NIDS;
    DcxPoolOut po;
    memset(&po, 0, sizeof(po));
    if (po_in != nullptr) {
        po = *po_in;
        if (!po.tickets || !po.cursor || !po.counts || !po.starts || !po.rows) return DCX_E_ARG;
        if (po.conf != nullptr && po.conf_cells == nullptr) return DCX_E_ARG;
        if (po.wc <= 0 || cells % po.wc != 0 || po.pool <= 0) return DCX_E_SHAPE;
    }
    const bool conf = po.conf != nullptr;
    const bool two = n_ids1 > 32;
    const int npix = 32;
    const int tiles = (cells + npix - 1) / npix;
    const long items = (long)batch * tiles;
    if (items > 0x7fffffffL) return DCX_E_SHAPE;
    const float4* a4 = reinterpret_cast<const float4*>(act);
    const float4* wl = reinterpret_cast<const float4*>(w_loc);
    const float4* wi = reinterpret_cast<const float4*>(w_ids);
#define DCX_TAIL_LAUNCH_PF(NT, IT, CF, PF)                                                                               \
    hipLaunchKernelGGL((dcx_tail_kernel<NT, IT, CF, PF>), dim3((unsigned)items), dim3(256), 0, s, a4, 128, cells, wl, b_loc, wi, b_ids, \
                       ids_cout_pad, n_ids1, tiles, dust_bin, codes, loc_argmax, ids_argmax, po, dcx_tail_fence_mode())
    const bool small = items < dcx_device_cu_count();
#define DCX_TAIL_LAUNCH(NT, IT, CF) do { if (small) DCX_TAIL_LAUNCH_PF(NT, IT, CF, kTailPFSmall); else DCX_TAIL_LAUNCH_PF(NT, IT, CF, kTailPF); } while (0)
    if (two) { if (conf) DCX_TAIL_LAUNCH(1, 2, true); else DCX_TAIL_LAUNCH(1, 2, false); }
    else     { if (conf) DCX_TAIL_LAUNCH(1, 1, true); else DCX_TAIL_LAUNCH(1, 1, false); }
#undef DCX_TAIL_LAUNCH
#undef DCX_TAIL_LAUNCH_PF
    return (int)hipGetLastError();
}
```

deepcharuco_amd/inference.py:

```python
from __future__ import annotations

import ctypes as _ctypes
import warnings
from typing import List, Optional

import numpy as np
import torch

from . import _lib
from .imgproc import _opencv, bgr2gray
from .models._handles import require_cuda, unwrap
from .models.model_utils import extract_patches, pre_bgr_image, pred_to_keypoints
from .models.net import dcModel, lModel
from .models.refinenet import RefineNet, lRefineNet
from .pnp import (solve_pnp_batch_device, solve_pnp_device, solve_pnp_host, solve_pnp_pool, solve_pnp_ransac_batch_device,
                  solve_pnp_ransac_device, solve_pnp_ransac_host, solve_pnp_ransac_pool, unpack_poses, unpack_ransac)

__all__ = ["load_models", "infer_image", "infer_image_staged", "infer_batch", "infer_batch_device", "unpack_results", "packed_len",
           "solve_pnp", "solve_pnp_batch", "solve_pnp_submit", "set_deterministic", "InferenceModel", "calibrate_xcd",
           "set_xcd_weights", "get_xcd_weights", "solve_pnp_host", "solve_pnp_device", "solve_pnp_batch_device", "solve_pnp_pool",
           "unpack_poses", "solve_pnp_ransac_host", "solve_pnp_ransac_device", "solve_pnp_ransac_batch_device",
           "solve_pnp_ransac_pool", "unpack_ransac"]

DEFAULT_KMAX = 64


def load_models(deepc_ckpt: str, refinenet_ckpt: Optional[str] = None, n_ids: int = 16, device="cuda"):
    deepc = lModel.load_from_checkpoint(deepc_ckpt, dcModel=dcModel(n_ids))
    deepc.eval()
    deepc.to(device)
    refinenet = None
    if refinenet_ckpt is not None:
        refinenet = lRefineNet.load_from_checkpoint(refinenet_ckpt, refinenet=RefineNet())
        refinenet.eval()
        refinenet.to(device)
    return deepc, refinenet


def _cv2_solvepnp():
    try:
        import cv2
    except ImportError as e:
        raise ImportError("solve_pnp needs OpenCV (cv2.solvePnP), which is not installed") from e
    return cv2.solvePnP


def _pnp_points(keypoints, col_count, row_count, square_len):
    inn_rc = np.arange(1, row_count)
    inn_cc = np.arange(1, col_count)
    object_points = np.zeros(((col_count - 1) * (row_count - 1), 3), np.float32)
    object_points[:, :2] = np.array(np.meshgrid(inn_rc, inn_cc)).reshape((2, -1)).T * square_len
    image_points = keypoints[:, :2].astype(np.float32)
    return object_points[keypoints[:, 2].astype(int)], image_points


def solve_pnp(keypoints, col_count, row_count, square_len, camera_matrix, dist_coeffs):
    if keypoints.shape[0] < 4:
        return False, None, None
    object_points_found, image_points = _pnp_points(keypoints, col_count, row_count, square_len)
    return _cv2_solvepnp()(object_points_found, image_points, camera_matrix, dist_coeffs)


_pnp_pools: dict = {}


def _pool(workers: Optional[int]):
    import concurrent.futures as cf
    import os
    n = int(workers) if workers else min(32, os.cpu_count() or 1)
    pool = _pnp_pools.get(n)
    if pool is None:
        pool = _pnp_pools[n] = cf.ThreadPoolExecutor(max_workers=n, thread_name_prefix="dcx-pnp")
    return pool


def solve_pnp_submit(keypoints_list, col_count, row_count, square_len, camera_matrix, dist_coeffs, workers: Optional[int] = None):
    import concurrent.futures as cf
    fn = _cv2_solvepnp()
    pool = _pool(workers)
    futs = []
    for kp in keypoints_list:
        kp = np.asarray(kp)
        if kp.ndim != 2 or kp.shape[0] < 4:
            f = cf.Future()
            f.set_result((False, None, None))
        else:
            obj, img = _pnp_points(kp, col_count, row_count, square_len)
            f = pool.submit(fn, obj, img, camera_matrix, dist_coeffs)
        futs.append(f)
    return futs


def solve_pnp_batch(keypoints_list, col_count, row_count, square_len, camera_matrix, dist_coeffs, workers: Optional[int] = None):
    return [f.result() for f in solve_pnp_submit(keypoints_list, col_count, row_count, square_len, camera_matrix,
                                                dist_coeffs, workers)]



def set_deterministic(enabled: bool = True) -> None:
    _lib.check(_lib.lib().dcx_set_deterministic(1 if enabled else 0), "dcx_set_deterministic")
    from .graph import clear_graph_cache
    clear_graph_cache()


def calibrate_xcd(device="cuda", rounds: int = 8) -> List[float]:
    dev = require_cuda(device)
    w = (_ctypes.c_float * 8)()
    with torch.cuda.device(dev):
        torch.cuda.synchronize()
        _lib.check(_lib.lib().dcx_calibrate_xcd(int(rounds), w, _lib.current_stream()), "dcx_calibrate_xcd")
    from .graph import clear_graph_cache
    clear_graph_cache()
    return [float(v) for v in w]


def set_xcd_weights(weights=None, device="cuda") -> None:
    dev = require_cuda(device)
    arr = None if weights is None else (_ctypes.c_float * 8)(*[float(v) for v in weights])
    with torch.cuda.device(dev):
        _lib.check(_lib.lib().dcx_set_xcd_weights(arr), "dcx_set_xcd_weights")
    from .graph import clear_graph_cache
    clear_graph_cache()


def get_xcd_weights(device="cuda") -> List[float]:
    dev = require_cuda(device)
    w = (_ctypes.c_float * 8)()
    with torch.cuda.device(dev):
        _lib.check(_lib.lib().dcx_get_xcd_weights(w), "dcx_get_xcd_weights")
    return [float(v) for v in w]


PIXEL_FORMATS = {"gray": 0, "opencv4": 1, "legacy14": 2}


def packed_len(batch: int, pool: int, conf: bool = False) -> int:
    return 2 * batch + (8 if conf else 6) * pool


def launch_pipeline(det, ref, frames_ptr: int, b: int, h: int, w: int, bpp: int, pix: int, dust_bin_ids: int, pool: int,
                    ws: torch.Tensor, out_ptr: int, conf: bool = False) -> None:
    counts_p, starts_p, rows_p = out_ptr, out_ptr + 4 * b, out_ptr + 8 * b
    xy_p = rows_p + 16 * pool
    conf_p = xy_p + 8 * pool
    _lib.check(_lib.lib().dcx_infer_batch(det.handle, ref.handle if ref else None, frames_ptr, h * w * bpp, w * bpp, pix, b, h, w,
                                          dust_bin_ids, pool, ws.data_ptr(), ws.numel(), counts_p, starts_p, rows_p,
                                          xy_p if ref else None, conf_p if conf else None, _lib.current_stream()), "dcx_infer_batch")


def infer_batch_device(frames: torch.Tensor, dust_bin_ids: int, deepc, refinenet=None, kmax: int = DEFAULT_KMAX,
                       out: Optional[torch.Tensor] = None, ws: Optional[torch.Tensor] = None, pool: Optional[int] = None,
                       conf: bool = False, bgr_variant: str = "opencv4") -> torch.Tensor:
    det, ref = unwrap(deepc), unwrap(refinenet)
    dev = det.device
    if (not isinstance(frames, torch.Tensor) or frames.device != dev or frames.dtype != torch.uint8 or not frames.is_contiguous()
            or not (frames.ndim == 3 or (frames.ndim == 4 and frames.shape[3] == 3))):
        raise ValueError("frames must be a contiguous (B,H,W) gray or (B,H,W,3) BGR uint8 tensor on the model's GPU")
    b, h, w = frames.shape[:3]
    bpp = 1 if frames.ndim == 3 else 3
    if bgr_variant not in ("opencv4", "legacy14"):
        raise ValueError(f"unknown BGR->gray variant {bgr_variant!r}")
    pix = PIXEL_FORMATS["gray" if bpp == 1 else bgr_variant]
    if pool is None:
        pool = b * kmax
    if pool <= 0:
        raise ValueError("pool must be positive")
    L = _lib.lib()
    with torch.cuda.device(dev):
        nbytes = L.dcx_pipeline_workspace_bytes(det.handle, ref.handle if ref else None, b, h, w, pool)
        if nbytes == 0:
            raise ValueError("bad batch/shape for dcx_pipeline_workspace_bytes")
        if ws is None:
            ws = det._ws.get("pipe", dev, nbytes)
        elif ws.device != dev or ws.dtype != torch.uint8 or not ws.is_contiguous() or ws.numel() < nbytes:
            raise ValueError(f"ws must be a contiguous uint8 tensor of >= {nbytes} bytes on {dev}")
        n_i32 = packed_len(b, pool, conf)
        if out is None:
            out = torch.empty((n_i32,), dtype=torch.int32, device=dev)
        elif out.device != dev or out.dtype != torch.int32 or out.numel() != n_i32 or not out.is_contiguous():
            raise ValueError(f"out must be a contiguous int32 tensor of {n_i32} elements on {dev}")
        launch_pipeline(det, ref, frames.data_ptr(), b, h, w, bpp, pix, dust_bin_ids, pool, ws, out.data_ptr(), conf)
    return out


def unpack_results(packed: np.ndarray, batch: int, pool: int, refined: bool, conf: bool = False):
    packed = np.asarray(packed, dtype=np.int32)
    counts = packed[:batch]
    head = packed[:2 * batch].tolist()
    rows = packed[2 * batch:2 * batch + 4 * pool].reshape(pool, 4)
    xy = packed[2 * batch + 4 * pool:2 * batch + 6 * pool].view(np.float32).reshape(pool, 2)
    cf = packed[2 * batch + 6 * pool:2 * batch + 8 * pool].view(np.float32).reshape(pool, 2) if conf else None
    res: List[Optional[np.ndarray]] = []
    confs: List[Optional[np.ndarray]] = []
    for b in range(batch):
        k, s0 = head[b], head[batch + b]
        if k == 0:
            res.append(np.array([]))
            confs.append(np.zeros((0, 2), np.float32))
            continue
        if s0 + k > pool:
            res.append(None)
            confs.append(None)
            continue
        rb = rows[s0:s0 + k]
        order = rb[:, 2].argsort(kind="stable")
        a = np.empty((k, 3), np.float64 if refined else np.int64)
        a[:, 0:2] = xy[s0:s0 + k] if refined else rb[:, 0:2]
        a[:, 2] = rb[:, 2]
        res.append(a[order])
        if conf:
            confs.append(cf[s0:s0 + k][order].copy())
    if conf:
        return res, counts.copy(), confs
    return res, counts.copy()


def _to_device_frames(frames, dev):
    if isinstance(frames, torch.Tensor):
        d = frames
    else:
        frames = np.ascontiguousarray(frames, dtype=np.uint8)
        d = torch.from_numpy(frames)
    if d.dtype != torch.uint8 or not (d.ndim == 3 or (d.ndim == 4 and d.shape[3] == 3)):
        raise ValueError("expected (B,H,W) uint8 gray frames or (B,H,W,3) uint8 BGR frames")
    return d.to(dev).contiguous()


def infer_batch(frames, dust_bin_ids: int, deepc, refinenet=None, kmax: int = DEFAULT_KMAX, pool: Optional[int] = None,
                conf: bool = False, bgr_variant: str = "opencv4"):
    det = unwrap(deepc)
    d_frames = _to_device_frames(frames, det.device)
    b = d_frames.shape[0]
    if pool is None:
        pool = b * kmax
    while True:
        packed = infer_batch_device(d_frames, dust_bin_ids, deepc, refinenet, pool=pool, conf=conf, bgr_variant=bgr_variant).cpu().numpy()
        out = unpack_results(packed, b, pool, refinenet is not None, conf)
        need = int(out[1].astype(np.int64).sum())
        if need <= pool:
            return (out[0], out[2]) if conf else out[0]
        warnings.warn(f"the batch produced {need} corners > pool={pool}; re-running with pool={need}")
        pool = need


_graph_state = {"enabled": None, "warned": False}
_graph_mod = [None]
_cuda_seen = [False]


def _graphs_enabled() -> bool:
    if _graph_state["enabled"] is None:
        import os
        _graph_state["enabled"] = os.environ.get("DCX_GRAPH", "1") not in ("", "0")
    return bool(_graph_state["enabled"])


def infer_image(img: np.ndarray, dust_bin_ids: int, deepc, refinenet=None, draw_pred: bool = False, device="cuda"):
    if device != "cuda":
        require_cuda(device)
    elif not _cuda_seen[0]:
        require_cuda(device)
        _cuda_seen[0] = True
    if not isinstance(img, np.ndarray) or img.ndim != 3 or img.shape[2] != 3 or img.dtype != np.uint8:
        raise ValueError("expected a (H,W,3) uint8 BGR image")
    if draw_pred:
        return infer_image_staged(img, dust_bin_ids, deepc, refinenet, True, device)
    keypoints = None
    frame = bgr2gray(img)[None] if _opencv() else img[None]
    G = _graph_mod[0]
    if G is None:
        from . import graph as G
        _graph_mod[0] = G
    graphs_usable, cached_pipeline = G.graphs_usable, G.cached_pipeline
    if _graphs_enabled() and graphs_usable():
        try:
            for attempt in (0, 1):
                pipe = cached_pipeline(dust_bin_ids, deepc, refinenet, img.shape[0], img.shape[1], bgr=frame.ndim == 4)
                try:
                    keypoints = pipe.run(frame)[0]
                    break
                except ReferenceError:
                    continue
        except (_lib.DcxError, ValueError):
            raise
        except RuntimeError as e:
            if not _graph_state["warned"]:
                warnings.warn(f"hipGraph capture failed ({e}); falling back to eager kernel launches")
                _graph_state["warned"] = True
            _graph_state["enabled"] = False
    if keypoints is None:
        keypoints = infer_batch(frame, dust_bin_ids, deepc, refinenet)[0]
    return keypoints, img


def infer_image_staged(img: np.ndarray, dust_bin_ids: int, deepc, refinenet=None, draw_pred: bool = False,
                       device="cuda"):
    require_cuda(device)
    img_gray = bgr2gray(img)
    img_gray = pre_bgr_image(img_gray)
    img_gray = torch.tensor(img_gray, device=device)
    loc_hat, ids_hat = deepc.infer_image(img_gray)
    keypoints, ids_found = pred_to_keypoints(loc_hat, ids_hat, dust_bin_ids)
    if draw_pred:
        img = (draw_inner_corners(img, keypoints.cpu().numpy(), ids_found.cpu().numpy(), radius=3, draw_ids=True, color=(0, 0, 255))
               if ids_found.shape[0] else img.copy())
    if ids_found.shape[0] == 0:
        return np.array([]), img
    if refinenet is not None:
        patches = extract_patches(img_gray, keypoints)
        keypoints, _ = refinenet.infer_patches(patches, keypoints)
    keypoints = keypoints.cpu().numpy()
    ids_found = ids_found.cpu().numpy()
    if draw_pred and refinenet is not None:
        img = draw_inner_corners(img, keypoints, ids_found, draw_ids=False, radius=1, color=(0, 255, 255))
    keypoints = np.array([[k[0], k[1], idx] for k, idx in sorted(zip(keypoints, ids_found), key=lambda x: x[1])])
    return keypoints, img


def draw_inner_corners(img: np.ndarray, corners: np.ndarray, ids: np.ndarray, draw_ids: bool = False, radius: int = 2,
                       color=(0, 0, 255)) -> np.ndarray:
    try:
        import cv2
    except ImportError as e:
        raise ImportError("draw_pred=True needs OpenCV for drawing, which is not installed") from e
    assert img.ndim == 3 and img.shape[-1] == 3
    out = img.copy()
    font, thickness = cv2.FONT_HERSHEY_COMPLEX_SMALL, 1
    for corner, idx in zip(corners, ids):
        c = np.round(corner).astype(int)
        if c[0] > out.shape[1] or c[1] > out.shape[0]:
            continue
        cv2.circle(out, (int(c[0]), int(c[1])), radius=radius, color=color, thickness=thickness)
        if draw_ids:
            (tw, th), _ = cv2.getTextSize(str(idx), font, .5, thickness)
            cv2.putText(out, str(idx), (int(c[0]) - tw // 2 - 7, int(c[1]) + th // 2 - 3), font, .45, (0, 255, 0), thickness)
    return out


class InferenceModel:

    def __init__(self, deepc_ckpt: str, refinenet_ckpt: Optional[str] = None, n_ids: int = 16, device="cuda"):
        self.n_ids = n_ids
        self.device = device
        self.deepc, self.refinenet = load_models(deepc_ckpt, refinenet_ckpt, n_ids, device)

    def infer_image(self, img: np.ndarray, draw_pred: bool = False):
        return infer_image(img, self.n_ids, self.deepc, self.refinenet, draw_pred, self.device)

    def infer_batch(self, frames: np.ndarray, kmax: int = DEFAULT_KMAX, conf: bool = False):
        return infer_batch(frames, self.n_ids, self.deepc, self.refinenet, kmax, conf=conf)
```

include/deepcharuco_amd.h:

```cpp
#ifndef DEEPCHARUCO_AMD_H
#define DEEPCHARUCO_AMD_H

#include <stddef.h>
#include <stdint.h>

#ifdef __cplusplus
extern "C" {
#endif

#define DCX_E_ARG      (-1)
#define DCX_E_SHAPE    (-2)
#define DCX_E_WS       (-3)
#define DCX_E_NIDS     (-4)

typedef struct dcx_detector dcx_detector;
typedef struct dcx_refiner  dcx_refiner;

const char* dcx_version(void);
const char* dcx_error_string(int code);

int dcx_detector_create(dcx_detector** out, const float* const* h_tensors, int n_tensors, int n_ids);
int dcx_detector_destroy(dcx_detector* det);
int dcx_refiner_create(dcx_refiner** out, const float* const* h_tensors, int n_tensors);
int dcx_refiner_destroy(dcx_refiner* rf);

size_t dcx_detector_workspace_bytes(const dcx_detector* det, int batch, int height, int width);
size_t dcx_refiner_workspace_bytes(const dcx_refiner* rf, int max_patches);

int dcx_bgr2gray(const uint8_t* d_bgr, long frame_stride, int pitch, int batch, int height, int width,
                 uint8_t* d_gray, void* stream);
int dcx_bgr2gray_legacy14(const uint8_t* d_bgr, long frame_stride, int pitch, int batch, int height, int width,
                          uint8_t* d_gray, void* stream);

int dcx_pre_image(const uint8_t* d_gray, float* d_out, size_t n, void* stream);

int dcx_detector_forward(const dcx_detector* det,
                         const uint8_t* d_frames_u8, long frame_stride, int pitch,
                         const float* d_images_f32,
                         int batch, int height, int width,
                         void* d_ws, size_t ws_bytes,
                         float* d_loc_nchw, float* d_ids_nchw, void* stream);

int dcx_detector_decode(const dcx_detector* det, int batch, int height, int width,
                        void* d_ws, int dust_bin, int kmax,
                        int32_t* d_counts, int32_t* d_rows,
                        int32_t* d_loc_argmax, int32_t* d_ids_argmax, void* stream);
int dcx_pred_to_keypoints(const float* d_loc_nchw, const float* d_ids_nchw,
                          int batch, int n_loc, int n_ids1, int hc, int wc,
                          int dust_bin, int kmax,
                          int32_t* d_counts, int32_t* d_rows,
                          int32_t* d_loc_argmax, int32_t* d_ids_argmax, void* stream);
int dcx_label_to_keypoints(const long long* d_loc, const long long* d_ids, int batch, int hc, int wc, int dust_bin, int kmax,
                           int32_t* d_counts, int32_t* d_rows, int32_t* d_codes, int32_t* d_bad, void* stream);

int dcx_build_patch_table(const int32_t* d_counts, const int32_t* d_rows, int batch, int kmax,
                          int32_t* d_table, int32_t* d_total, void* stream);

int dcx_extract_patches_u8(const uint8_t* d_frames, long frame_stride, int pitch, int height, int width,
                           const int32_t* d_table, const int32_t* d_total, int max_patches,
                           float* d_patches, void* stream);
int dcx_extract_patches_f32(const float* d_images, int height, int width,
                            const int32_t* d_table, const int32_t* d_total, int max_patches,
                            float* d_patches, void* stream);

int dcx_refiner_forward(const dcx_refiner* rf, const float* d_patches, int max_patches,
                        const int32_t* d_total, const int32_t* d_table,
                        void* d_ws, size_t ws_bytes,
                        int32_t* d_corners, float* d_xy, float* d_heat, void* stream);

int dcx_argmax2d(const float* d_x, int k, int h, int w, int32_t* d_out, void* stream);

#define DCX_PIX_GRAY8          0
#define DCX_PIX_BGR8           1
#define DCX_PIX_BGR8_LEGACY14  2
size_t dcx_pipeline_workspace_bytes(const dcx_detector* det, const dcx_refiner* rf,
                                    int batch, int height, int width, int pool);
int dcx_infer_batch(const dcx_detector* det, const dcx_refiner* rf,
                    const uint8_t* d_frames_u8, long frame_stride, int pitch, int pixel_format,
                    int batch, int height, int width, int dust_bin, int pool,
                    void* d_ws, size_t ws_bytes,
                    int32_t* d_counts, int32_t* d_starts, int32_t* d_rows, float* d_xy, float* d_conf, void* stream);
int dcx_stream_synchronize(void* stream);

#define DCX_PNP_OK          0
#define DCX_PNP_TOO_FEW     1
#define DCX_PNP_TRUNCATED   2
#define DCX_PNP_BAD_ID      3
#define DCX_PNP_DEGENERATE  4
#define DCX_PNP_NONFINITE   5
int dcx_solve_pnp_pool(const int32_t* d_counts, const int32_t* d_starts, const int32_t* d_rows,
                       const float* d_xy , int batch, int pool,
                       int col_count, int row_count, double square_len,
                       const double* h_camera9, const double* h_dist, int n_dist,
                       int32_t* d_status, double* d_pose ,
                       void* stream);

#define DCX_PNP_NO_CONSENSUS 6
size_t dcx_solve_pnp_ransac_workspace_bytes(int batch, int pool, int iterations);
int dcx_solve_pnp_ransac_pool(const int32_t* d_counts, const int32_t* d_starts, const int32_t* d_rows,
                              const float* d_xy , int batch, int pool,
                              int col_count, int row_count, double square_len,
                              const double* h_camera9, const double* h_dist, int n_dist,
                              int iterations, double reproj_error, int min_inliers, unsigned seed,
                              void* d_workspace, size_t workspace_bytes,
                              int32_t* d_status, double* d_pose , int32_t* d_info ,
                              uint8_t* d_inliers , void* stream);

#define DCX_CALIB_OK          0
#define DCX_CALIB_NO_VIEWS    1
#define DCX_CALIB_DEGENERATE  2
#define DCX_CALIB_NONFINITE   3
size_t dcx_calibrate_workspace_bytes(int batch);
int dcx_calibrate_pool(const int32_t* d_counts, const int32_t* d_starts, const int32_t* d_rows,
                       const float* d_xy , int batch, int pool,
                       int col_count, int row_count, double square_len, int image_width, int image_height,
                       void* d_workspace, size_t workspace_bytes,
                       int32_t* d_view_status , double* d_pose ,
                       double* h_result , void* stream);

int dcx_conv_layer(const float* d_in, int n, int cin, int hin, int win,
                   const float* h_weight_oihw, const float* h_bias,
                   const float* h_bn_gamma, const float* h_bn_beta,
                   const float* h_bn_mean, const float* h_bn_var,
                   int cout, int ksize, int pad, int ups, int pool, int relu,
                   float* d_out, void* stream);
int dcx_nchw_to_c4(const float* d_nchw, int n, int c, int h, int w, float* d_c4, void* stream);
int dcx_c4_to_nchw(const float* d_c4, int n, int c, int h, int w, float* d_nchw, void* stream);

int dcx_set_timing(int enabled);
int dcx_get_timing(void);
int dcx_last_timings(float* h_ms4);

const char* dcx_conv_pick_name(int n, int cin, int ho, int wo, int cout, int ks, int pool, int epi);
const char* dcx_conv_pick_name_ups(int n, int cin, int ho, int wo, int cout, int ks, int pool, int epi, int ups);

int dcx_set_deterministic(int enabled);
int dcx_get_deterministic(void);

int dcx_set_tail_fence(int enabled);
int dcx_get_tail_fence(void);

int dcx_calibrate_xcd(int rounds, float* w8_out, void* stream);
int dcx_set_xcd_weights(const float* w8);
int dcx_get_xcd_weights(float* w8);

int dcx_profile_enable(int enabled);
int dcx_profile_enabled(void);
int dcx_profile_count(void);
int dcx_profile_filter(int kernel_id);
int dcx_profile_sample(int every);
int dcx_profile_fetch(int* kernel_ids, int* n_images, int* limited, double* flops_per_image, float* ms,
                      int max_records);
const char* dcx_profile_kernel_name(int kernel_id);
int dcx_profile_clocks(float* ghz, int max_records);
int dcx_profile_probe_words(int record, unsigned long long* out64);

#ifdef __cplusplus
}
#endif
#endif
```

Measured before the change: 10310 frames/s.

## Gate detector location head to cells flagged by the ids head

Splits the fused 512-channel head conv so the backbone now computes only the ids branch (convDa) densely. A new ids-tail kernel emits a candidate list of cells with a non-dust id. A gather kernel then packs each candidate's input window into small maps, the location branch (convPa) runs only on those maps, and a separate loc tail plus ordered compaction finish the outputs. A dense convPa fallback, sized from a device counter, runs when candidates overflow the cap. This is meant to cut most of the convPa work and its loc-head arithmetic, at the cost of extra kernel launches, gather traffic and device-side control words. It is enabled automatically when batch times cells reaches a threshold, and can be forced on or off through an env knob or API.

```diff
diff --git a/deepcharuco_amd/_lib.py b/deepcharuco_amd/_lib.py
--- a/deepcharuco_amd/_lib.py
+++ b/deepcharuco_amd/_lib.py
@@ -84,6 +84,9 @@
     "dcx_get_xcd_weights": (_i, [C.POINTER(C.c_float)]),
     "dcx_set_tail_fence": (_i, [_i]),
     "dcx_get_tail_fence": (_i, []),
+    "dcx_set_loc_gate": (_i, [_i]),
+    "dcx_get_loc_gate": (_i, []),
+    "dcx_last_loc_gate": (_i, [C.POINTER(_i), C.POINTER(_i)]),
     "dcx_profile_enable": (_i, [_i]),
     "dcx_profile_count": (_i, []),
     "dcx_profile_filter": (_i, [_i]),
diff --git a/deepcharuco_amd/csrc/dcx_api.hip b/deepcharuco_amd/csrc/dcx_api.hip
--- a/deepcharuco_amd/csrc/dcx_api.hip
+++ b/deepcharuco_amd/csrc/dcx_api.hip
@@ -1,4 +1,5 @@
 #include "dcx_common.h"
+#include "dcx_conv_shared.h"
 
 #include <math.h>
 #include <stdlib.h>
@@ -194,6 +195,7 @@
     DevLayer first;
     DevLayer enc[7];
     DevLayer heads_a;
+    DevLayer head_pa, head_da;
     DevLayer head_loc, head_ids;
 };
 
@@ -301,6 +303,8 @@
         rc = make_layer(HostConv{w.data(), b.data(), g.data(), be.data(), mu.data(), var.data()}, 128, 512, 3,
                         &d->heads_a);
     }
+    if (rc == 0) rc = make_layer(hc(48, true), 128, 256, 3, &d->head_pa);
+    if (rc == 0) rc = make_layer(hc(56, true), 128, 256, 3, &d->head_da);
     if (rc == 0) rc = make_layer(hc(54, false), 256, 65, 1, &d->head_loc);
     if (rc == 0) rc = make_layer(hc(62, false), 256, n_ids + 1, 1, &d->head_ids);
     if (rc != 0) { dcx_detector_destroy(d); return rc; }
@@ -312,7 +316,7 @@
     if (!d) return 0;
     free_layer(d->first);
     for (auto& l : d->enc) free_layer(l);
-    free_layer(d->heads_a); free_layer(d->head_loc); free_layer(d->head_ids);
+    free_layer(d->heads_a); free_layer(d->head_pa); free_layer(d->head_da); free_layer(d->head_loc); free_layer(d->head_ids);
     delete d;
     return 0;
 }
@@ -325,7 +329,8 @@
 namespace {
 int detector_run(const dcx_detector* det, const uint8_t* d_frames_u8, long frame_stride, int pitch, int pix,
                  const float* d_images_f32, int batch, int height, int width, void* d_ws, size_t ws_bytes,
-                 bool with_heads, float* d_loc_nchw, float* d_ids_nchw, int32_t* zero_words, int n_zero, void* stream);
+                 bool with_heads, float* d_loc_nchw, float* d_ids_nchw, int32_t* zero_words, int n_zero, void* stream,
+                 bool da_only = false);
 }
 
 extern "C" int dcx_detector_forward(const dcx_detector* det, const uint8_t* d_frames_u8, long frame_stride, int pitch,
@@ -338,7 +343,8 @@
 namespace {
 int detector_run(const dcx_detector* det, const uint8_t* d_frames_u8, long frame_stride, int pitch, int pix,
                  const float* d_images_f32, int batch, int height, int width, void* d_ws, size_t ws_bytes,
-                 bool with_heads, float* d_loc_nchw, float* d_ids_nchw, int32_t* zero_words, int n_zero, void* stream) {
+                 bool with_heads, float* d_loc_nchw, float* d_ids_nchw, int32_t* zero_words, int n_zero, void* stream,
+                 bool da_only) {
     if (!det || !d_ws) return DCX_E_ARG;
     if ((d_frames_u8 == nullptr) == (d_images_f32 == nullptr)) return DCX_E_ARG;
     if (batch <= 0 || height < 8 || width < 8) return DCX_E_SHAPE;
@@ -373,6 +379,11 @@
         float* t = src; src = dst; dst = t;
     }
     const int hc = h / 8, wc = w / 8;
+    if (da_only) {
+        DcxConvArgs a = conv_args(det->head_da, src, batch, 32, 0, hc, wc, 0, 1, dst, 128, nullptr);
+        a.out_cq_off = 64;
+        return dcx_launch_conv_mfma(a, 3, 0, DCX_EPI_BNRELU, s);
+    }
     {
         DcxConvArgs a = conv_args(det->heads_a, src, batch, 32, 0, hc, wc, 0, 1, dst, 128, nullptr);
         rc = dcx_launch_conv_mfma(a, 3, 0, DCX_EPI_BNRELU, s);
@@ -533,12 +544,56 @@
     size_t off = 0;
     L.det = off; off = align_up(off + det_layout(det->n_ids, b, h, w).total, 256);
     L.table = off; off = align_up(off + (size_t)pool * 16, 256);
-    L.ctrl_words = 64 + b;
+    L.ctrl_words = DCX_CTRL_TICKETS + b;
     L.ctrl = off; off = align_up(off + (size_t)L.ctrl_words * 4, 256);
     L.ref = off; off = align_up(off + (rf ? ref_layout(pool).total : 0), 256);
     L.total = off;
     return L;
 }
+
+struct GateWs { size_t cin, cout, cand; int cap, maps; bool fits; };
+GateWs gate_layout(int b, int h, int w) {
+    GateWs G;
+    const size_t cells = (size_t)(h / 8) * (w / 8), bc = (size_t)b * cells;
+    const size_t capq = bc >> DCX_LOC_GATE_CAP_SHIFT;
+    G.cap = (int)(capq < 8 ? 8 : capq > (1u << 24) ? (1u << 24) : capq);
+    G.maps = (G.cap + DCX_GATE_PER_MAP - 1) / DCX_GATE_PER_MAP;
+    size_t off = align_up(bc * 128 * 16, 256);
+    G.cin = off;  off = align_up(off + (size_t)G.maps * 32 * DCX_GATE_MAP_H * DCX_GATE_MAP_W * 16, 256);
+    G.cout = off; off = align_up(off + (size_t)G.maps * 64 * DCX_GATE_OUT_H * DCX_GATE_OUT_W * 16, 256);
+    G.cand = off; off = align_up(off + (size_t)G.cap * 4, 256);
+    G.fits = off <= (size_t)b * 64 * h * w * 4 && bc <= 0x3fffffffu;
+    return G;
+}
+
+constexpr long kGateMinCells = 19200;
+int g_loc_gate = -2;
+int loc_gate_mode() {
+    if (g_loc_gate == -2) { const int v = dcx_env_knob(DCX_KNOB_LOC_GATE); g_loc_gate = v == 0 || v == 1 ? v : -1; }
+    return g_loc_gate;
+}
+bool use_gated_tail(int b, int h, int w) {
+    if (!gate_layout(b, h, w).fits) return false;
+    const int mode = loc_gate_mode();
+    return mode >= 0 ? mode == 1 : (long)b * (h / 8) * (w / 8) >= kGateMinCells;
+}
+const int32_t* g_gate_ctrl = nullptr;
+bool g_gate_enqueued = false;
+}
+
+extern "C" int dcx_set_loc_gate(int mode) { g_loc_gate = mode == 0 || mode == 1 ? mode : -1; return 0; }
+extern "C" int dcx_get_loc_gate(void) { return loc_gate_mode(); }
+extern "C" int dcx_last_loc_gate(int* h_candidates, int* h_form) {
+    if (!h_candidates || !h_form) return DCX_E_ARG;
+    if (g_gate_ctrl == nullptr) return DCX_E_ARG;
+    *h_candidates = -1;
+    *h_form = DCX_LOC_GATE_DENSE;
+    if (!g_gate_enqueued) return 0;
+    int32_t words[DCX_CTRL_FORM + 1];
+    DCX_CHECK_HIP(hipMemcpy(words, g_gate_ctrl, sizeof(words), hipMemcpyDeviceToHost));
+    *h_candidates = words[DCX_CTRL_CAND];
+    *h_form = words[DCX_CTRL_FORM] == 1 ? DCX_LOC_GATE_GATED : DCX_LOC_GATE_FALLBACK;
+    return 0;
 }
 
 extern "C" size_t dcx_pipeline_workspace_bytes(const dcx_detector* det, const dcx_refiner* rf, int batch, int height,
@@ -557,25 +612,68 @@
     int rc = timing ? timing_mark(0, s) : 0;
     if (rc) return rc;
     int32_t* ctrl = (int32_t*)(ws + L.ctrl);
+    const bool gated = use_gated_tail(batch, height, width);
+    g_gate_ctrl = ctrl;
+    g_gate_enqueued = gated;
     rc = detector_run(det, d_frames_u8, frame_stride, pitch, pix, nullptr, batch, height, width, ws + L.det, L.table - L.det,
-                      false, nullptr, nullptr, ctrl, L.ctrl_words, stream);
+                      false, nullptr, nullptr, ctrl, L.ctrl_words, stream, gated);
     if (rc) return rc;
     if (timing && (rc = timing_mark(1, s))) return rc;
     int32_t* table = (int32_t*)(ws + L.table);
     {
         const DetWs D = det_layout(det->n_ids, batch, height, width);
         const int hc = height / 8, wc = width / 8;
-        const float* act = (const float*)(ws + L.det + D.buf0);
+        float* act = (float*)(ws + L.det + D.buf0);
         int32_t* codes = (int32_t*)(ws + L.det + D.codes);
         DcxPoolOut po;
-        po.tickets = ctrl + 64; po.cursor = ctrl; po.counts = d_counts; po.starts = d_starts; po.rows = d_rows;
+        memset(&po, 0, sizeof(po));
+        po.tickets = ctrl + DCX_CTRL_TICKETS; po.cursor = ctrl + DCX_CTRL_CURSOR; po.counts = d_counts; po.starts = d_starts; po.rows = d_rows;
         po.table = rf ? table : nullptr; po.conf = d_conf; po.conf_cells = (float*)(ws + L.det + D.conf);
         po.wc = wc; po.pool = pool;
-        const int pt = dcx_prof_begin(DCX_PROF_TAIL, batch, s);
-        rc = dcx_launch_tail(act, batch, hc * wc, det->head_loc.w, det->head_loc.bias, det->head_ids.w, det->head_ids.bias,
-                             det->head_ids.cout_pad, det->n_ids + 1, dust_bin, codes, nullptr, nullptr, &po, s);
-        if (rc) return rc;
-        if ((rc = dcx_prof_end(pt, s))) return rc;
+        if (!gated) {
+            const int pt = dcx_prof_begin(DCX_PROF_TAIL, batch, s);
+            rc = dcx_launch_tail(act, batch, hc * wc, det->head_loc.w, det->head_loc.bias, det->head_ids.w, det->head_ids.bias,
+                                 det->head_ids.cout_pad, det->n_ids + 1, dust_bin, codes, nullptr, nullptr, &po, s);
+            if (rc) return rc;
+            if ((rc = dcx_prof_end(pt, s))) return rc;
+        } else {
+            const GateWs G = gate_layout(batch, height, width);
+            const float* conv4b = (const float*)(ws + L.det + D.buf1);
+            float* cin = (float*)(ws + L.det + D.buf0 + G.cin);
+            float* cout = (float*)(ws + L.det + D.buf0 + G.cout);
+            po.cand = (int32_t*)(ws + L.det + D.buf0 + G.cand); po.cand_cursor = ctrl + DCX_CTRL_CAND; po.cand_cap = G.cap;
+            int pt = dcx_prof_begin(DCX_PROF_TAIL_IDS, batch, s);
+            rc = dcx_launch_tail_ids(act, batch, hc * wc, det->head_ids.w, det->head_ids.bias, det->head_ids.cout_pad, det->n_ids + 1,
+                                     dust_bin, codes, &po, s);
+            if (rc) return rc;
+            if ((rc = dcx_prof_end(pt, s))) return rc;
+            pt = dcx_prof_begin(DCX_PROF_LOC_GATHER, batch, s);
+            rc = dcx_launch_loc_gather(conv4b, batch, hc, wc, &po, ctrl, cin, s);
+            if (rc) return rc;
+            if ((rc = dcx_prof_end(pt, s))) return rc;
+            {
+                DcxConvArgs a = conv_args(det->head_pa, cin, G.maps, 32, 0, DCX_GATE_MAP_H, DCX_GATE_MAP_W, 0, 0, cout, 64, ctrl + DCX_CTRL_MAPS);
+                const long expect = ((long)batch * det->n_ids + DCX_GATE_PER_MAP - 1) / DCX_GATE_PER_MAP;
+                a.n_hint = (int)(expect < G.maps ? expect : G.maps);
+                dcx_prof_next_images(a.n_hint);
+                rc = dcx_launch_conv_mfma(a, 3, 0, DCX_EPI_BNRELU, s);
+                if (rc) return rc;
+            }
+            {
+                DcxConvArgs a = conv_args(det->head_pa, conv4b, batch, 32, 0, hc, wc, 0, 1, act, 128, ctrl + DCX_CTRL_DENSE_N);
+                dcx_prof_next_images(0);
+                rc = dcx_launch_conv_mfma(a, 3, 0, DCX_EPI_BNRELU, s);
+                if (rc) return rc;
+            }
+            pt = dcx_prof_begin(DCX_PROF_TAIL_LOC, batch, s);
+            rc = dcx_launch_tail_loc(act, cout, batch, hc * wc, det->head_loc.w, det->head_loc.bias, dust_bin, codes, &po, s);
+            if (rc) return rc;
+            if ((rc = dcx_prof_end(pt, s))) return rc;
+            pt = dcx_prof_begin(DCX_PROF_TAIL_COMPACT, batch, s);
+            rc = dcx_launch_tail_compact(codes, batch, hc * wc, dust_bin, &po, s);
+            if (rc) return rc;
+            if ((rc = dcx_prof_end(pt, s))) return rc;
+        }
     }
     if (timing && (rc = timing_mark(2, s))) return rc;
     if (rf == nullptr) return timing ? timing_mark(3, s) : 0;
diff --git a/deepcharuco_amd/csrc/dcx_common.h b/deepcharuco_amd/csrc/dcx_common.h
--- a/deepcharuco_amd/csrc/dcx_common.h
+++ b/deepcharuco_amd/csrc/dcx_common.h
@@ -59,9 +59,11 @@
 int dcx_conv_cout_pad(int cout);
 int dcx_conv_heat_tiles(int ho, int wo, int ups);
 
-enum { DCX_PROF_CONV1A = 100, DCX_PROF_PATCHES = 101, DCX_PROF_TAIL = 102, DCX_PROF_FINALIZE = 103 };
+enum { DCX_PROF_CONV1A = 100, DCX_PROF_PATCHES = 101, DCX_PROF_TAIL = 102, DCX_PROF_FINALIZE = 103,
+       DCX_PROF_TAIL_IDS = 104, DCX_PROF_LOC_GATHER = 105, DCX_PROF_TAIL_LOC = 106, DCX_PROF_TAIL_COMPACT = 107 };
 int dcx_prof_begin(int kernel_id, int n, hipStream_t s);
 int dcx_prof_end(int token, hipStream_t s);
+void dcx_prof_next_images(int n);
 
 
 int dcx_launch_conv1_u8(const uint8_t* frames, long frame_stride, int pitch, int pix, int n, int h, int w, int pad,
@@ -88,10 +90,27 @@
     float* conf;
     float* conf_cells;
     int wc, pool;
+    int32_t* cand;
+    int32_t* cand_cursor;
+    int cand_cap;
 };
 int dcx_launch_tail(const float* act_c4_512, int batch, int cells, const float* w_loc, const float* b_loc,
                     const float* w_ids, const float* b_ids, int ids_cout_pad, int n_ids1, int dust_bin,
                     int32_t* codes, int32_t* loc_argmax, int32_t* ids_argmax, const DcxPoolOut* po, hipStream_t s);
+enum { DCX_GATE_MAP_H = 8, DCX_GATE_MAP_W = 16, DCX_GATE_PER_MAP = 8, DCX_GATE_OUT_H = 6, DCX_GATE_OUT_W = 14 };
+enum { DCX_CTRL_CURSOR = 0,
+       DCX_CTRL_CAND = 1,
+       DCX_CTRL_MAPS = 2,
+       DCX_CTRL_DENSE_N = 3,
+       DCX_CTRL_FORM = 4,
+       DCX_CTRL_TICKETS = 64 };
+int dcx_launch_tail_ids(const float* act_c4_512, int batch, int cells, const float* w_ids, const float* b_ids, int ids_cout_pad,
+                        int n_ids1, int dust_bin, int32_t* codes, const DcxPoolOut* po, hipStream_t s);
+int dcx_launch_loc_gather(const float* conv4b_c4, int batch, int hc, int wc, const DcxPoolOut* po, int32_t* ctrl, float* compact_in,
+                          hipStream_t s);
+int dcx_launch_tail_loc(const float* act_c4_512, const float* compact_out, int batch, int cells, const float* w_loc, const float* b_loc,
+                        int dust_bin, int32_t* codes, const DcxPoolOut* po, hipStream_t s);
+int dcx_launch_tail_compact(const int32_t* codes, int batch, int cells, int dust_bin, const DcxPoolOut* po, hipStream_t s);
 int dcx_launch_compact(const int32_t* codes, int batch, int hc, int wc, int dust_bin, int kmax, int32_t* counts,
                        int32_t* rows, hipStream_t s);
 int dcx_launch_conv1_patches_u8(const uint8_t* frames, long frame_stride, int pitch, int pix, int h, int w, const int32_t* table,
diff --git a/deepcharuco_amd/csrc/dcx_conv_mfma.hip b/deepcharuco_amd/csrc/dcx_conv_mfma.hip
--- a/deepcharuco_amd/csrc/dcx_conv_mfma.hip
+++ b/deepcharuco_amd/csrc/dcx_conv_mfma.hip
@@ -157,6 +157,7 @@
 std::vector<ProfRec> g_recs;
 std::vector<hipEvent_t> g_pool;
 size_t g_pool_used = 0;
+thread_local int g_prof_next_n = -1;
 
 hipEvent_t prof_event() {
     if (g_pool_used == g_pool.size()) {
@@ -197,6 +198,10 @@
         case DCX_PROF_PATCHES: return "dcx_conv1_patches_kernel (RefineNet conv1a + patch gather)";
         case DCX_PROF_TAIL: return "dcx_tail_kernel (1x1 heads + arg-max + compaction)";
         case DCX_PROF_FINALIZE: return "dcx_refine_finalize_kernel";
+        case DCX_PROF_TAIL_IDS: return "dcx_tail_ids_kernel (gated: ids head + candidate list)";
+        case DCX_PROF_LOC_GATHER: return "dcx_loc_gather_kernel (gated: candidates' convPa windows)";
+        case DCX_PROF_TAIL_LOC: return "dcx_tail_loc_kernel (gated: loc head on the candidates)";
+        case DCX_PROF_TAIL_COMPACT: return "dcx_tail_compact_kernel (gated: ordered compaction)";
         default: break;
     }
     return id >= 0 && id < n ? kCfgs[id].name : "?";
@@ -213,6 +218,7 @@
     g_recs.push_back(r);
     return r.slot;
 }
+void dcx_prof_next_images(int n) { g_prof_next_n = n; }
 int dcx_prof_end(int token, hipStream_t stream) {
     if (token < 0 || token >= (int)g_recs.size()) return 0;
     DCX_CHECK_HIP(hipEventRecord(g_recs[token].e1, stream));
@@ -285,6 +291,7 @@
         {"DCX_W2HS_ROUNDS", 1},
         {"DCX_W2PS", 7},
         {"DCX_PROBE_U0", 0},
+        {"DCX_LOC_GATE", -1},
     };
     if (!knobs[k].read) { const char* e = getenv(knobs[k].name); knobs[k].value = e ? atoi(e) : knobs[k].unset; knobs[k].read = true; }
     return knobs[k].value;
@@ -439,12 +446,14 @@
                              a.ups == 0 && a.pad == 1,
                              (a.ups == 1 && a.pad == 1 && ks == 3 && a.w_ups2w != nullptr) ? 1 : 0);
     if (c == nullptr) return DCX_E_SHAPE;
+    const int prof_n = g_prof_next_n;
+    g_prof_next_n = -1;
     if (!g_prof || (g_prof_filter >= 0 && g_prof_filter != (int)(c - kCfgs))) return c->launch(a, stream);
     if (g_prof_every > 1 && (g_prof_seen++ % g_prof_every) != 0) return c->launch(a, stream);
     ProfRec r;
     r.kernel_id = (int)(c - kCfgs);
-    r.n = a.n;
-    r.limited = a.n_limit != nullptr;
+    r.n = prof_n >= 0 ? prof_n : a.n;
+    r.limited = prof_n >= 0 ? 0 : a.n_limit != nullptr;
     r.flops_per_image = 2.0 * a.cout_real * a.cin * ks * ks
                       * (double)a.ho * a.wo;
     r.e0 = prof_event();
diff --git a/deepcharuco_amd/csrc/dcx_conv_shared.h b/deepcharuco_amd/csrc/dcx_conv_shared.h
--- a/deepcharuco_amd/csrc/dcx_conv_shared.h
+++ b/deepcharuco_amd/csrc/dcx_conv_shared.h
@@ -121,7 +121,7 @@
 int dcx_device_cu_count();
 int dcx_fill_xcd_cum(DcxConvArgs& a);
 enum DcxKnob { DCX_KNOB_DETERMINISTIC, DCX_KNOB_XCD_WALK, DCX_KNOB_OCC, DCX_KNOB_CT_OUTER, DCX_KNOB_W2HS, DCX_KNOB_W2HS_ROUNDS,
-               DCX_KNOB_W2PS, DCX_KNOB_PROBE_U0, DCX_KNOB_COUNT };
+               DCX_KNOB_W2PS, DCX_KNOB_PROBE_U0, DCX_KNOB_LOC_GATE, DCX_KNOB_COUNT };
 int dcx_env_knob(DcxKnob k);
 
 template <void (*KERNEL)(const DcxConvArgs)>
diff --git a/deepcharuco_amd/csrc/dcx_tail.hip b/deepcharuco_amd/csrc/dcx_tail.hip
--- a/deepcharuco_amd/csrc/dcx_tail.hip
+++ b/deepcharuco_amd/csrc/dcx_tail.hip
@@ -18,7 +18,7 @@
 __device__ __forceinline__ int dcx_ld_agent(const int32_t* p) {
     return __hip_atomic_load(const_cast<int32_t*>(p), __ATOMIC_RELAXED, __HIP_MEMORY_SCOPE_AGENT);
 }
-template <bool CONF>
+template <bool CONF, bool LIST = false>
 __device__ __forceinline__ void dcx_tail_compact_frame(const int32_t* codes, int cells, int dust_bin, int b, const DcxPoolOut& po,
                                                        int* s_cnt , int* s_bcast) {
     const int tid = threadIdx.x, lane = tid & 63, wave = tid >> 6;
@@ -61,9 +61,11 @@
         if (sc == 0) {
             if (nsuper == 1) total = acc;
             if (tid == 0) {
-                const int st = atomicAdd(po.cursor, total);
-                po.counts[b] = total;
-                po.starts[b] = st;
+                const int st = atomicAdd(LIST ? po.cand_cursor : po.cursor, total);
+                if (!LIST) {
+                    po.counts[b] = total;
+                    po.starts[b] = st;
+                }
                 *s_bcast = st;
             }
             __syncthreads();
@@ -73,7 +75,9 @@
         for (int c = 0; c < 8; ++c) {
             if ((code[c] >> 8) != dust_bin) {
                 const int pos = start + run + base[c] + __popcll(m[c] & ((1ull << lane) - 1ull));
-                if (pos < po.pool) {
+                if (LIST) {
+                    if (pos < po.cand_cap) po.cand[pos] = b * cells + (sc * 2048 + c * 256 + tid);
+                } else if (pos < po.pool) {
                     const int cell = sc * 2048 + c * 256 + tid;
                     const int la = code[c] & 255, ia = code[c] >> 8;
                     const int cy = cell / po.wc, cx = cell - cy * po.wc;
@@ -91,6 +95,72 @@
         }
         run += acc;
         __syncthreads();
+    }
+}
+
+template <bool CONF, int PF>
+__device__ __forceinline__ void dcx_tail_job(const float4* __restrict__ act, size_t a_off, size_t k_stride, const float4* __restrict__ wq,
+                                             int cout_pad, int m0, int n_valid, const float* __restrict__ bias,
+                                             float* rv, int* ri, float* rs) {
+    const int lane = threadIdx.x & 63, half = lane >> 5, l31 = lane & 31;
+    const size_t w_lane = (size_t)half * cout_pad + (m0 + l31);
+    const size_t w_stride = (size_t)2 * cout_pad;
+    dcx_t_f32x16 acc;
+#pragma unroll
+    for (int r = 0; r < 16; ++r) acc[r] = 0.f;
+    float4 aq[32 + PF], bq[32 + PF];
+#pragma unroll
+    for (int st = 0; st < PF; ++st) {
+        aq[st] = wq[w_lane + st * w_stride];
+        bq[st] = act[a_off + st * k_stride];
+    }
+#pragma unroll
+    for (int st = 0; st < 32; ++st) {
+        __builtin_amdgcn_sched_barrier(0);
+        if (st + PF < 32) {
+            aq[st + PF] = wq[w_lane + (st + PF) * w_stride];
+            bq[st + PF] = act[a_off + (st + PF) * k_stride];
+        }
+        __builtin_amdgcn_sched_barrier(0);
+        const float4 av = aq[st], bv = bq[st];
+#pragma unroll
+        for (int j = 0; j < 4; ++j) {
+            const float a1 = j == 0 ? av.x : j == 1 ? av.y : j == 2 ? av.z : av.w;
+            const float b1 = j == 0 ? bv.x : j == 1 ? bv.y : j == 2 ? bv.z : bv.w;
+            acc = __builtin_amdgcn_mfma_f32_32x32x2f32(a1, b1, acc, 0, 0, 0);
+        }
+    }
+    float best = -INFINITY;
+    int besti = 0x7fffffff;
+    float lv[16];
+#pragma unroll
+    for (int r = 0; r < 16; ++r) {
+        const int co = m0 + 8 * (r >> 2) + 4 * half + (r & 3);
+        lv[r] = -INFINITY;
+        if (co < n_valid) {
+            const float v = acc[r] + bias[co];
+            lv[r] = v;
+            if (v > best || besti == 0x7fffffff) { best = v; besti = co; }
+        }
+    }
+    float ssum = 0.f;
+    if (CONF && besti != 0x7fffffff) {
+#pragma unroll
+        for (int r = 0; r < 16; ++r) ssum += lv[r] == -INFINITY ? 0.f : expf(lv[r] - best);
+    }
+    const float ov = __shfl_xor(best, 32);
+    const int oi = __shfl_xor(besti, 32);
+    const float os = CONF ? __shfl_xor(ssum, 32) : 0.f;
+    const float mine = best;
+    if (oi != 0x7fffffff && (besti == 0x7fffffff || ov > best || (ov == best && oi < besti))) { best = ov; besti = oi; }
+    if (half == 0) {
+        rv[l31] = best;
+        ri[l31] = besti;
+        if (CONF) {
+            const float a = ssum == 0.f ? 0.f : ssum * expf(mine - best);
+            const float c = os == 0.f ? 0.f : os * expf(ov - best);
+            rs[l31] = a + c;
+        }
     }
 }
 
@@ -251,6 +321,148 @@
     dcx_tail_compact_frame<CONF>(codes, cells, dust_bin, b, po, s_cnt, &s_bcast);
 }
 
+
+
+template <int IDS_TILES, bool CONF, int PF = kTailPF>
+__global__ __launch_bounds__(256) void dcx_tail_ids_kernel(const float4* __restrict__ act, int act_cq_total, int cells,
+                                                            const float4* __restrict__ w_ids, const float* __restrict__ b_ids,
+                                                            int ids_cout_pad, int n_ids1, int tiles_per_frame, int dust_bin,
+                                                            int32_t* codes, DcxPoolOut po, int fence) {
+#if defined(__HIP_DEVICE_COMPILE__) && !defined(__gfx950__) && !defined(__gfx942__)
+#error "dcx_tail_ids_kernel uses dcx_tail_kernel's fence-free hand-off: see there"
+#endif
+    __shared__ float red_v[IDS_TILES][128];
+    __shared__ int red_i[IDS_TILES][128];
+    __shared__ float red_s[CONF ? IDS_TILES : 1][128];
+    __shared__ int s_cnt[32];
+    __shared__ int s_bcast, s_last;
+    const int tid = threadIdx.x, lane = tid & 63, wave = tid >> 6;
+    const int item = blockIdx.x;
+    const int b = item / tiles_per_frame;
+    const int cell0 = (item - b * tiles_per_frame) * 128;
+    const int pix = min(cell0 + wave * 32 + (lane & 31), cells - 1);
+    const size_t a_off = ((size_t)b * act_cq_total + 64 + (lane >> 5)) * (size_t)cells + pix;
+    if (cell0 + wave * 32 < cells) {
+        for (int job = 0; job < IDS_TILES; ++job)
+            dcx_tail_job<CONF, PF>(act, a_off, (size_t)2 * cells, w_ids, ids_cout_pad, job * 32, n_ids1, b_ids, red_v[job] + wave * 32,
+                                   red_i[job] + wave * 32, red_s[CONF ? job : 0] + wave * 32);
+    }
+    __syncthreads();
+    if (tid < 128 && cell0 + tid < cells) {
+        float iv = red_v[0][tid];
+        int ia = red_i[0][tid];
+        if (IDS_TILES > 1) {
+            const int ti = red_i[1][tid];
+            if (ti != 0x7fffffff && red_v[1][tid] > iv) { iv = red_v[1][tid]; ia = ti; }
+        }
+        const size_t o = (size_t)b * cells + cell0 + tid;
+        if (CONF) {
+            float si = red_s[0][tid] * expf(red_v[0][tid] - iv);
+            if (IDS_TILES > 1 && red_i[1][tid] != 0x7fffffff) si += red_s[1][tid] * expf(red_v[1][tid] - iv);
+            __hip_atomic_store(po.conf_cells + 2 * o + 1, 1.0f / si, __ATOMIC_RELAXED, __HIP_MEMORY_SCOPE_AGENT);
+        }
+        __hip_atomic_store(codes + o, ia << 8, __ATOMIC_RELAXED, __HIP_MEMORY_SCOPE_AGENT);
+    }
+    if (fence) __threadfence();
+    else asm volatile("s_waitcnt vmcnt(0)" ::: "memory");
+    __syncthreads();
+    if (tid == 0) s_last = __hip_atomic_fetch_add(&po.tickets[b], 1, fence ? __ATOMIC_ACQ_REL : __ATOMIC_RELAXED, __HIP_MEMORY_SCOPE_AGENT) == tiles_per_frame - 1;
+    __syncthreads();
+    if (!s_last) return;
+    if (fence) __threadfence();
+    dcx_tail_compact_frame<false, true>(codes, cells, dust_bin, b, po, s_cnt, &s_bcast);
+}
+
+__global__ __launch_bounds__(256) void dcx_loc_gather_kernel(const float4* __restrict__ src, int batch, int hc, int wc, const int32_t* __restrict__ cand,
+                                                              int cand_cap, int32_t* ctrl, float4* __restrict__ cin) {
+    const int tid = threadIdx.x;
+    const int n_cand = ctrl[DCX_CTRL_CAND];
+    const bool gated = n_cand <= cand_cap;
+    if (blockIdx.x == 0 && tid == 0) {
+        ctrl[DCX_CTRL_MAPS] = gated ? (n_cand + DCX_GATE_PER_MAP - 1) / DCX_GATE_PER_MAP : 0;
+        ctrl[DCX_CTRL_DENSE_N] = gated ? 0 : batch;
+        ctrl[DCX_CTRL_FORM] = gated ? 1 : 2;
+    }
+    if (!gated) return;
+    const int cells = hc * wc;
+    for (int e = blockIdx.x; e < n_cand; e += gridDim.x) {
+        const int o = cand[e];
+        const int b = o / cells, cell = o - b * cells;
+        const int cy = cell / wc, cx = cell - cy * wc;
+        const int y0 = (cy & ~1) - 1, x0 = (cx & ~1) - 1;
+        const int map = e / DCX_GATE_PER_MAP, k = e - map * DCX_GATE_PER_MAP;
+        const int r0 = 4 * (k >> 2), c0 = 4 * (k & 3);
+#pragma unroll
+        for (int i = tid; i < 32 * 16; i += 256) {
+            const int cq = i >> 4, py = (i >> 2) & 3, px = i & 3;
+            const int y = y0 + py, x = x0 + px;
+            float4 v = make_float4(0.f, 0.f, 0.f, 0.f);
+            if ((unsigned)y < (unsigned)hc && (unsigned)x < (unsigned)wc) v = src[(((size_t)b * 32 + cq) * hc + y) * wc + x];
+            cin[(((size_t)map * 32 + cq) * DCX_GATE_MAP_H + r0 + py) * DCX_GATE_MAP_W + c0 + px] = v;
+        }
+    }
+}
+
+template <bool CONF, int PF = kTailPF>
+__global__ __launch_bounds__(256) void dcx_tail_loc_kernel(const float4* __restrict__ act, const float4* __restrict__ cmp, int batch, int cells, int wc,
+                                                            const float4* __restrict__ w_loc, const float* __restrict__ b_loc, int dust_bin,
+                                                            int32_t* codes, DcxPoolOut po) {
+    __shared__ float red_v[3][32];
+    __shared__ int red_i[3][32];
+    __shared__ float red_s[CONF ? 3 : 1][32];
+    const int tid = threadIdx.x, lane = tid & 63, wave = tid >> 6;
+    const int half = lane >> 5, l31 = lane & 31;
+    const int n_cand = dcx_ld_agent(po.cand_cursor);
+    const bool dense = n_cand > po.cand_cap;
+    const int total = dense ? batch * cells : n_cand;
+    constexpr int PLANE = DCX_GATE_OUT_H * DCX_GATE_OUT_W;
+    for (int e0 = blockIdx.x * 32; e0 < total; e0 += gridDim.x * 32) {
+        const int e = min(e0 + l31, total - 1);
+        const int o = dense ? e : po.cand[e];
+        const int b = o / cells, cell = o - b * cells;
+        size_t a_off, k_stride;
+        if (dense) {
+            a_off = ((size_t)b * 128 + half) * (size_t)cells + cell;
+            k_stride = (size_t)2 * cells;
+        } else {
+            const int cy = cell / wc, cx = cell - cy * wc;
+            const int map = e / DCX_GATE_PER_MAP, k = e - map * DCX_GATE_PER_MAP;
+            a_off = ((size_t)map * 64 + half) * PLANE + (4 * (k >> 2) + (cy & 1)) * DCX_GATE_OUT_W + 4 * (k & 3) + (cx & 1);
+            k_stride = 2 * PLANE;
+        }
+        if (wave < 3)
+            dcx_tail_job<CONF, PF>(dense ? act : cmp, a_off, k_stride, w_loc, 128, wave * 32, 65, b_loc, red_v[wave], red_i[wave], red_s[CONF ? wave : 0]);
+        __syncthreads();
+        if (tid < 32 && e0 + tid < total) {
+            float lv = red_v[0][tid];
+            int la = red_i[0][tid];
+#pragma unroll
+            for (int t = 1; t < 3; ++t) {
+                const int ti = red_i[t][tid];
+                if (ti != 0x7fffffff && red_v[t][tid] > lv) { lv = red_v[t][tid]; la = ti; }
+            }
+            if (CONF) {
+                float sl = 0.f;
+#pragma unroll
+                for (int t = 0; t < 3; ++t)
+                    if (red_i[t][tid] != 0x7fffffff) sl += red_s[t][tid] * expf(red_v[t][tid] - lv);
+                __hip_atomic_store(po.conf_cells + 2 * (size_t)o, 1.0f / sl, __ATOMIC_RELAXED, __HIP_MEMORY_SCOPE_AGENT);
+            }
+            int ia = dcx_ld_agent(codes + o) >> 8;
+            if (la == 64) ia = dust_bin;
+            __hip_atomic_store(codes + o, la | (ia << 8), __ATOMIC_RELAXED, __HIP_MEMORY_SCOPE_AGENT);
+        }
+        __syncthreads();
+    }
+}
+
+template <bool CONF>
+__global__ __launch_bounds__(256) void dcx_tail_compact_kernel(const int32_t* codes, int cells, int dust_bin, DcxPoolOut po) {
+    __shared__ int s_cnt[32];
+    __shared__ int s_bcast;
+    dcx_tail_compact_frame<CONF>(codes, cells, dust_bin, blockIdx.x, po, s_cnt, &s_bcast);
+}
+
 }
 
 static int g_tail_fence = -1;
@@ -295,3 +507,69 @@
 #undef DCX_TAIL_LAUNCH_PF
     return (int)hipGetLastError();
 }
+
+static int dcx_gate_po(const DcxPoolOut* po_in, int batch, int cells, DcxPoolOut* po) {
+    if (!po_in) return DCX_E_ARG;
+    *po = *po_in;
+    if (!po->tickets || !po->cursor || !po->counts || !po->starts || !po->rows || !po->cand || !po->cand_cursor) return DCX_E_ARG;
+    if (po->conf != nullptr && po->conf_cells == nullptr) return DCX_E_ARG;
+    if (batch <= 0 || cells <= 0 || po->wc <= 0 || cells % po->wc != 0 || po->pool <= 0 || po->cand_cap <= 0) return DCX_E_SHAPE;
+    if ((long)batch * cells > 0x7fffffffL) return DCX_E_SHAPE;
+    return 0;
+}
+
+int dcx_launch_tail_ids(const float* act, int batch, int cells, const float* w_ids, const float* b_ids, int ids_cout_pad, int n_ids1,
+                        int dust_bin, int32_t* codes, const DcxPoolOut* po_in, hipStream_t s) {
+    if (!act || !w_ids || !b_ids || !codes) return DCX_E_ARG;
+    if (n_ids1 < 2 || n_ids1 > 64 || ids_cout_pad < n_ids1) return DCX_E_SHAPE;
+    if (dust_bin < 0 || dust_bin > 255) return DCX_E_NIDS;
+    DcxPoolOut po;
+    if (const int rc = dcx_gate_po(po_in, batch, cells, &po)) return rc;
+    const int tiles = (cells + 127) / 128;
+    const long items = (long)batch * tiles;
+    const float4* a4 = reinterpret_cast<const float4*>(act);
+    const float4* wi = reinterpret_cast<const float4*>(w_ids);
+#define DCX_TAIL_IDS_LAUNCH(IT, CF) \
+    hipLaunchKernelGGL((dcx_tail_ids_kernel<IT, CF>), dim3((unsigned)items), dim3(256), 0, s, a4, 128, cells, wi, b_ids, ids_cout_pad, n_ids1, \
+                       tiles, dust_bin, codes, po, dcx_tail_fence_mode())
+    if (n_ids1 > 32) { if (po.conf) DCX_TAIL_IDS_LAUNCH(2, true); else DCX_TAIL_IDS_LAUNCH(2, false); }
+    else             { if (po.conf) DCX_TAIL_IDS_LAUNCH(1, true); else DCX_TAIL_IDS_LAUNCH(1, false); }
+#undef DCX_TAIL_IDS_LAUNCH
+    return (int)hipGetLastError();
+}
+
+int dcx_launch_loc_gather(const float* conv4b, int batch, int hc, int wc, const DcxPoolOut* po_in, int32_t* ctrl, float* cin, hipStream_t s) {
+    if (!conv4b || !ctrl || !cin) return DCX_E_ARG;
+    DcxPoolOut po;
+    if (const int rc = dcx_gate_po(po_in, batch, hc * wc, &po)) return rc;
+    if (po.cand_cursor != ctrl + DCX_CTRL_CAND) return DCX_E_ARG;
+    const int grid = po.cand_cap < 1024 ? po.cand_cap : 1024;
+    hipLaunchKernelGGL(dcx_loc_gather_kernel, dim3(grid), dim3(256), 0, s, reinterpret_cast<const float4*>(conv4b), batch, hc, wc, po.cand,
+                       po.cand_cap, ctrl, reinterpret_cast<float4*>(cin));
+    return (int)hipGetLastError();
+}
+
+int dcx_launch_tail_loc(const float* act, const float* cmp, int batch, int cells, const float* w_loc, const float* b_loc, int dust_bin,
+                        int32_t* codes, const DcxPoolOut* po_in, hipStream_t s) {
+    if (!act || !cmp || !w_loc || !b_loc || !codes) return DCX_E_ARG;
+    if (dust_bin < 0 || dust_bin > 255) return DCX_E_NIDS;
+    DcxPoolOut po;
+    if (const int rc = dcx_gate_po(po_in, batch, cells, &po)) return rc;
+    const long items = ((long)batch * cells + 31) / 32;
+    const int grid = (int)(items < 4L * dcx_device_cu_count() ? items : 4L * dcx_device_cu_count());
+    const float4* a4 = reinterpret_cast<const float4*>(act);
+    const float4* c4 = reinterpret_cast<const float4*>(cmp);
+    const float4* wl = reinterpret_cast<const float4*>(w_loc);
+    if (po.conf) hipLaunchKernelGGL((dcx_tail_loc_kernel<true>), dim3(grid), dim3(256), 0, s, a4, c4, batch, cells, po.wc, wl, b_loc, dust_bin, codes, po);
+    else hipLaunchKernelGGL((dcx_tail_loc_kernel<false>), dim3(grid), dim3(256), 0, s, a4, c4, batch, cells, po.wc, wl, b_loc, dust_bin, codes, po);
+    return (int)hipGetLastError();
+}
+
+int dcx_launch_tail_compact(const int32_t* codes, int batch, int cells, int dust_bin, const DcxPoolOut* po_in, hipStream_t s) {
+    if (!codes) return DCX_E_ARG;
+    DcxPoolOut po;
+    if (const int rc = dcx_gate_po(po_in, batch, cells, &po)) return rc;
+    if (po.conf) hipLaunchKernelGGL((dcx_tail_compact_kernel<true>), dim3(batch), dim3(256), 0, s, codes, cells, dust_bin, po);
+    else hipLaunchKernelGGL((dcx_tail_compact_kernel<false>), dim3(batch), dim3(256), 0, s, codes, cells, dust_bin, po);
+    return (int)hipGetLastError();
+}
diff --git a/deepcharuco_amd/inference.py b/deepcharuco_amd/inference.py
--- a/deepcharuco_amd/inference.py
+++ b/deepcharuco_amd/inference.py
@@ -101,6 +101,24 @@
     _lib.check(_lib.lib().dcx_set_deterministic(1 if enabled else 0), "dcx_set_deterministic")
     from .graph import clear_graph_cache
     clear_graph_cache()
+
+
+def set_loc_gate(mode: Optional[str] = None) -> None:
+    modes = {None: -1, "auto": -1, "dense": 0, "gated": 1}
+    if mode not in modes:
+        raise ValueError(f"unknown tail form {mode!r}")
+    _lib.check(_lib.lib().dcx_set_loc_gate(modes[mode]), "dcx_set_loc_gate")
+    from .graph import clear_graph_cache
+    clear_graph_cache()
+
+
+def last_loc_gate(device="cuda"):
+    dev = require_cuda(device)
+    n, form = _ctypes.c_int(), _ctypes.c_int()
+    with torch.cuda.device(dev):
+        torch.cuda.synchronize(dev)
+        _lib.check(_lib.lib().dcx_last_loc_gate(_ctypes.byref(n), _ctypes.byref(form)), "dcx_last_loc_gate")
+    return n.value, ("dense", "gated", "fallback")[form.value]
 
 
 def calibrate_xcd(device="cuda", rounds: int = 8) -> List[float]:
diff --git a/include/deepcharuco_amd.h b/include/deepcharuco_amd.h
--- a/include/deepcharuco_amd.h
+++ b/include/deepcharuco_amd.h
@@ -140,6 +140,15 @@
 int dcx_set_tail_fence(int enabled);
 int dcx_get_tail_fence(void);
 
+#define DCX_LOC_GATE_CAP_SHIFT 2
+#define DCX_LOC_GATE_AUTO     (-1)
+#define DCX_LOC_GATE_DENSE    0
+#define DCX_LOC_GATE_GATED    1
+#define DCX_LOC_GATE_FALLBACK 2
+int dcx_set_loc_gate(int mode);
+int dcx_get_loc_gate(void);
+int dcx_last_loc_gate(int* h_candidates, int* h_form);
+
 int dcx_calibrate_xcd(int rounds, float* w8_out, void* stream);
 int dcx_set_xcd_weights(const float* w8);
 int dcx_get_xcd_weights(float* w8);
```

Result: faster. 10440 frames/s, median of 5 (+1.3%).
